# decastyle/discovering-path-tracer

Measured on AMD Instinct MI355X. Metric: Mrays/s at 1920x1080x8spp, box.obj BVH, higher is better.
Workload: dtype f32

## Files before the change

discovering-path-tracer_amd/csrc/kernels/render.h:

```cpp

__device__ __forceinline__ unsigned long long wave_sum(unsigned long long v) {
#pragma unroll
  for (int off = 32; off > 0; off >>= 1) v += __shfl_xor(v, off, 64);
  return v;
}

__device__ __forceinline__ void flush_traced(const RenderParams& P, const Ctr& c, int lane) {
  const unsigned long long v0 = wave_sum(c.rays), v1 = wave_sum(c.srays), v2 = wave_sum(c.nodes),
                           v3_ = wave_sum(c.leaves), v4 = wave_sum(c.prim);
  if (lane == 0) {
    atomicAdd(&P.stats[4], v0);
    atomicAdd(&P.stats[5], v1);
    atomicAdd(&P.stats[6], v2);
    atomicAdd(&P.stats[7], v3_);
    atomicAdd(&P.stats[8], v4);
  }
}

__device__ __forceinline__ void fold_constant(const RenderParams& P, float* acc, int spl, int j) {
  if (P.n_batches == 0) return;
#pragma unroll
  for (int ch = 0; ch < 4; ++ch) {
    if (ch % spl != j) continue;
    const float k = ch < 3 ? 0.0f : 1.0f;
    if (acc[ch] == k || (P.first_batch == 0 && __builtin_isfinite(acc[ch]))) {
      acc[ch] = k;
    } else {
      for (uint32_t t = 0; t < P.n_batches; ++t) {
        const uint32_t batch = P.first_batch + t;
        acc[ch] = (acc[ch] * (float)batch + k) / (float)(batch + 1u);
      }
    }
  }
}

__device__ __forceinline__ void store_lane(float4* px, const float* acc, int spl, int j) {
  float* a = (float*)px;
#pragma unroll
  for (int ch = 0; ch < 4; ++ch)
    if (ch % spl == j) a[ch] = acc[ch];
}

__device__ __forceinline__ void emit_lane(const RenderParams& P, bool active, size_t pix, int q, const float* acc,
                                          int spl, int j) {
  if (P.pack_out)
    store_lane(P.pack_out + (size_t)blockIdx.x * (size_t)(256 / spl) + (size_t)q, acc, spl, j);
  else if (active)
    store_lane(P.accum + pix, acc, spl, j);
}

__device__ __forceinline__ bool pixel_tight(const RenderParams& P, float ndcX0, float ndcY0) {
  if (P.n_cull_tight < 0) return true;
  bool tight = false;
#pragma unroll
  for (int r = 0; r < kMaxCullRects; ++r)
    tight = tight || (r < P.n_cull_tight && ndcX0 >= P.cull_tight[r][0] && ndcX0 <= P.cull_tight[r][1] &&
                      ndcY0 >= P.cull_tight[r][2] && ndcY0 <= P.cull_tight[r][3]);
  return tight;
}

#ifndef PT_PIX_PER_FILL
#define PT_PIX_PER_FILL 8
#endif
constexpr int kPixPerFill = PT_PIX_PER_FILL;
__device__ __forceinline__ int item_shift(int spl) { return 8 - __builtin_ctz((unsigned)spl); }
__device__ __forceinline__ void fill_culled(const RenderParams& P, const int2* __restrict__ org, int n, int block) {
  const int lg = item_shift(P.spl);
  const long long total = (long long)n << lg;
  for (int k = 0; k < kPixPerFill; ++k) {
    const long long g = ((long long)block * kPixPerFill + k) * 256 + threadIdx.x;
    if (g >= total) return;
    const int2 o = org[g >> lg];
    const int q = (int)g & ((1 << lg) - 1);
    const int px = o.x + (q & 15);
    const int py = o.y + (q >> 4);
    if (px >= P.width || py >= P.height) continue;
    float4* dst = P.accum + (size_t)py * (size_t)P.width + (size_t)px;
    float acc[4] = {0.0f, 0.0f, 0.0f, 0.0f};
    if (!(P.fresh && P.first_batch == 0)) {
      const float4 a = *dst;
      acc[0] = a.x; acc[1] = a.y; acc[2] = a.z; acc[3] = a.w;
    }
    fold_constant(P, acc, 1, 0);
    *dst = make_float4(acc[0], acc[1], acc[2], acc[3]);
  }
}

__device__ __forceinline__ bool tile_pixel(const RenderParams& P, int tile, int part, int q, size_t* pix) {
  const int spl = P.spl;
  int bx, by;
  tile_block(tile, P.blocks_x, &bx, &by);
  const int px = bx * 16 + q % 16;
  const int py = by * 16 + part * (16 / spl) + q / 16;
  *pix = (size_t)py * (size_t)P.width + (size_t)px;
  return px < P.width && py < P.height;
}

__device__ __forceinline__ void unpack_pixel(const RenderParams& P, float4* __restrict__ frame,
                                             const float4* __restrict__ src, size_t slot_f4,
                                             const int* __restrict__ table, long long g) {
  const int lg = item_shift(P.spl);
  const int4 e = ((const int4*)table)[g >> lg];
  const int q = (int)g & ((1 << lg) - 1);
  const int px = e.y + (q & 15), py = e.z + (q >> 4);
  if (px >= P.width || py >= P.height) return;
  frame[(size_t)py * (size_t)P.width + (size_t)px] =
      e.w >= 0 ? src[(size_t)e.x * slot_f4 + ((size_t)e.w << lg) + q] : make_float4(0.0f, 0.0f, 0.0f, 1.0f);
}

__device__ __forceinline__ void unpack_block(const RenderParams& P, int block) {
  const long long total = (long long)P.n_unpack * (256 / P.spl);
  for (int k = 0; k < kPixPerFill; ++k) {
    const long long g = ((long long)block * kPixPerFill + k) * 256 + threadIdx.x;
    if (g >= total) return;
    unpack_pixel(P, P.unpack_frame, P.unpack_src, (size_t)P.unpack_slot_f4, P.unpack_table, g);
  }
}

__device__ __forceinline__ float fold_one(float a, float c, uint32_t batch) {
  const float fb = (float)batch, fb1 = (float)(batch + 1u);
  if (a == 1.0f && c == 1.0f && batch < (1u << 24)) return 1.0f;
  const float x = a * fb + c;
  if (((batch + 1u) & batch) == 0u && batch + 1u != 0u) return x * (1.0f / fb1);
  return x / fb1;
}

#ifdef PT_WG_TRACE
constexpr int kWgTraceCap = 1 << 16;
__device__ unsigned long long g_wg_trace[kWgTraceCap][4];
#endif

template <bool STATS, bool LDS, bool CNT = false, int SWEEP = 0, bool MOMENTS = false, bool EXIT = false>
#ifndef PT_RENDER_MIN_BLOCKS
#define PT_RENDER_MIN_BLOCKS 5
#endif
__global__ __launch_bounds__(256, SWEEP || (LDS && !STATS) ? 6 : PT_RENDER_MIN_BLOCKS) void render_kernel(RenderParams P) {
  const int tid = (int)threadIdx.x;
  if ((P.items || P.pack_out) && (int)blockIdx.x >= P.n_items) {
    if (P.pack_out)
      unpack_block(P, (int)blockIdx.x - P.n_items);
    else
      fill_culled(P, P.culled_org, P.n_culled_items, (int)blockIdx.x - P.n_items);
    return;
  }
  const unsigned long long cost_t0 = P.cost_out ? wall_clock64() : 0ull;
  int gx0, gy0;
  bool tile_ok = true;
  int spl = P.spl;
  if (P.items_org) {
    const int2 o = P.items_org[blockIdx.x];
    gx0 = o.x & ((1 << kMixShift) - 1);
    gy0 = o.y;
    if (P.mix) spl = 1 << (o.x >> kMixShift);
  } else {
    const int item = (int)blockIdx.x;
    const int tile = rank_tile(P, item / spl);
    int bx, by;
    tile_block(tile, P.blocks_x, &bx, &by);
    gx0 = bx * 16;
    gy0 = by * 16 + (item % spl) * (16 / spl);
    tile_ok = tile < P.blocks_total;
  }
#ifdef PT_WG_TRACE
  const unsigned long long wg_t0 = wall_clock64();
#endif
  const int wave = tid >> 6, lane = tid & 63;
  static_assert(!SWEEP || (LDS && !STATS && !CNT), "the sweep walk is the plain LDS kernel's");
  constexpr int kQueue = SWEEP ? 0 : kCand;
  static_assert(!MOMENTS || (!STATS && !CNT), "moments: the plain kernels only");
  constexpr int kHand = MOMENTS ? 5 : 4;
  static_assert(kPark >= kHand, "the hand-off shares the parked state's area");
  __shared__ int cand_buf[4][kQueue + kPark][64];
  int* cand = &cand_buf[wave][0][lane];
  float* colw = (float*)&cand_buf[wave][kQueue][0];
  const int q = wave * (64 / spl) + lane / spl;
  const int j = lane % spl;
  const int px = gx0 + q % 16;
  const int py = gy0 + q / 16;
  const bool active = tile_ok && px < P.width && py < P.height;
  Ctr c = {0u, 0u, 0u, 0u, 0u};
  const int W = P.width, H = P.height;
  const float ndcX0 = (2.0f * (float)px / (float)W) - 1.0f;
  const float ndcY0 = (2.0f * (float)py / (float)H) - 1.0f;
  bool live = true;
  bool wg_live = true;
  if (P.n_cull >= 0) {
    const float wx0 = (2.0f * (float)gx0 / (float)W) - 1.0f, wx1 = (2.0f * (float)(gx0 + 15) / (float)W) - 1.0f;
    const float wy0 = (2.0f * (float)gy0 / (float)H) - 1.0f;
    const float wy1 = (2.0f * (float)(gy0 + 16 / spl - 1) / (float)H) - 1.0f;
    live = false;
    wg_live = false;
#pragma unroll
    for (int r = 0; r < kMaxCullRects; ++r) {
      live = live || (r < P.n_cull && ndcX0 >= P.cull[r][0] && ndcX0 <= P.cull[r][1] && ndcY0 >= P.cull[r][2] &&
                      ndcY0 <= P.cull[r][3]);
      wg_live = wg_live || (r < P.n_cull && wx1 >= P.cull[r][0] && wx0 <= P.cull[r][1] && wy1 >= P.cull[r][2] &&
                            wy0 <= P.cull[r][3]);
    }
  }
  const bool tight = STATS || pixel_tight(P, ndcX0, ndcY0);
  const size_t pix = (size_t)py * (size_t)W + (size_t)px;
  uint32_t nsamp = 0;
  if (active && (uint32_t)j < P.n_batches)
    nsamp = (P.n_batches - (uint32_t)j + (uint32_t)spl - 1) / (uint32_t)spl;
  float acc[4] = {0.0f, 0.0f, 0.0f, 0.0f};
  if (active && !(P.fresh && P.first_batch == 0)) {
    const float* a = (const float*)&P.accum[pix];
#pragma unroll
    for (int ch = 0; ch < 4; ++ch)
      if (ch % spl == j) acc[ch] = a[ch];
  }
  if (!live && active) fold_constant(P, acc, spl, j);
  float mom1 = 0.0f, mom2 = 0.0f;
  if constexpr (MOMENTS) {
    if (active && live && j == 0 && P.first_batch != 0) {
      const float2 m = P.moments[pix];
      mom1 = m.x;
      mom2 = m.y;
    }
  }
  if (!wg_live) {
    emit_lane(P, active, pix, q, acc, spl, j);
    return;
  }
  if (SWEEP) {
    extern __shared__ float4 lds_scene[];
    const SweepTable tb = {P.sweep, P.sweep_boxes, P.sweep_leaves};
    const int* slot = sweep_slots(tb);
    const int nt = 3 * P.sweep_leaves;
    for (int i = tid; i < nt; i += 256) lds_scene[i] = P.tris[3 * slot[i / 3] + i % 3];
    __syncthreads();
    P.tris = lds_scene;
    P.hit_tris = P.tris;
  } else if (LDS) {
    extern __shared__ float4 lds_scene[];
    const int nn = 2 * P.n_nodes, nt = 3 * P.n_tris;
    for (int i = tid; i < nn; i += 256) lds_scene[i] = P.nodes[i];
    for (int i = tid; i < nt; i += 256) lds_scene[nn + i] = P.tris[i];
    __syncthreads();
    P.nodes = lds_scene;
    P.tris = lds_scene + nn;
    P.hit_tris = P.tris;
  }
  {
    const v3 cpos = mk(P.cam_pos[0], P.cam_pos[1], P.cam_pos[2]);
    const v3 cdir = mk(P.cam_dir[0], P.cam_dir[1], P.cam_dir[2]);
    const float aspect = (float)W / (float)H;
    const v3 right = mk(P.cam_right[0], P.cam_right[1], P.cam_right[2]);
    const v3 up = mk(P.cam_upv[0], P.cam_upv[1], P.cam_upv[2]);
    const float tanFov = P.tan_fov;
    for (uint32_t base = 0; base < P.n_batches; base += (uint32_t)spl) {
     const uint32_t s = base + (uint32_t)j;
     float4 col4 = make_float4(0.0f, 0.0f, 0.0f, 1.0f);
     if (active && live && s < P.n_batches) {
      const uint32_t batch = (P.first_batch + P.seed_base) + s;
      const uint32_t seed = (batch * (uint32_t)H + (uint32_t)py) * (uint32_t)W + (uint32_t)px;
      uint32_t rng = seed;
      const float u1a = fmax_(1e-38f, rng_next(&rng));
      const float u2a = rng_next(&rng);
      const float u1j = fmax_(1e-38f, rng_next(&rng));
      const float u2j = rng_next(&rng);
      if (tight || u1a < P.cull_u0 || u1j < P.cull_u0) {
      float r = sqrt_(-2.0f * log_(u1a));
      float th = (2.0f * 0x1.921fb6p+1f) * u2a;
      float sn, cs;
      sincos_(th, &sn, &cs);
      const float ax = (r * cs) * 0.02f;
      const float ay = (r * sn) * 0.02f;
      const v3 origin = add(add(cpos, muls(right, ax)), muls(up, ay));
      r = sqrt_(-2.0f * log_(u1j));
      th = (2.0f * 0x1.921fb6p+1f) * u2j;
      sincos_(th, &sn, &cs);
      const float jx = r * cs, jy = r * sn;
      const float ndcX = ndcX0 + (jx * 0.5f) / (float)W;
      const float ndcY = ndcY0 + (jy * 0.5f) / (float)H;
      const v3 bdir = normalize(sub(add(cdir, muls(neg(right), (ndcX * tanFov) * aspect)), muls(up, ndcY * tanFov)));
      const v3 focal = add(cpos, muls(bdir, 3.0f));
      const v3 dir = normalize(sub(focal, origin));
      v3 col;
      if (CNT) c.prim++;
      if (STATS || LDS)
        col = path_trace<STATS, !LDS, CNT, SWEEP>(P, origin, dir, seed, c, cand);
      else
        col = path_trace_fused<CNT, EXIT>(P, origin, dir, seed, cand, c);
      col4 = make_float4(col.x, col.y, col.z, 1.0f);
      }
     }
     if (spl == 1) {
      if (active && live) {
        const uint32_t batch = P.first_batch + base;
        acc[0] = fold_one(acc[0], col4.x, batch);
        acc[1] = fold_one(acc[1], col4.y, batch);
        acc[2] = fold_one(acc[2], col4.z, batch);
        acc[3] = fold_one(acc[3], col4.w, batch);
        if constexpr (MOMENTS) {
          const float L = ptdn::lum(col4.x, col4.y, col4.z);
          mom1 = fold_one(mom1, L, batch);
          mom2 = fold_one(mom2, L * L, batch);
        }
      }
      continue;
     }
     colw[lane] = col4.x;
     colw[64 + lane] = col4.y;
     colw[128 + lane] = col4.z;
     colw[192 + lane] = col4.w;
     if constexpr (MOMENTS) colw[256 + lane] = ptdn::lum(col4.x, col4.y, col4.z);
     __builtin_amdgcn_fence(__ATOMIC_RELEASE, "wavefront");
     __builtin_amdgcn_wave_barrier();
     __builtin_amdgcn_fence(__ATOMIC_ACQUIRE, "wavefront");
     if (active && live) {
      const uint32_t m = min((uint32_t)spl, P.n_batches - base);
      const int first_lane = lane - j;
      for (uint32_t t = 0; t < m; ++t) {
        const uint32_t batch = P.first_batch + base + t;
        const float* cc = colw + first_lane + (int)t;
#pragma unroll
        for (int ch = 0; ch < 4; ++ch)
          if (ch % spl == j) acc[ch] = fold_one(acc[ch], cc[ch * 64], batch);
        if constexpr (MOMENTS) {
          if (j == 0) {
            const float L = cc[256];
            mom1 = fold_one(mom1, L, batch);
            mom2 = fold_one(mom2, L * L, batch);
          }
        }
      }
     }
     __builtin_amdgcn_fence(__ATOMIC_RELEASE, "wavefront");
     __builtin_amdgcn_wave_barrier();
     __builtin_amdgcn_fence(__ATOMIC_ACQUIRE, "wavefront");
    }
  }
  emit_lane(P, active, pix, q, acc, spl, j);
  if constexpr (MOMENTS) {
    if (active && live && j == 0) P.moments[pix] = make_float2(mom1, mom2);
  }
  if (!STATS && P.cost_out && lane == 0) {
    const int part_row = (gy0 + wave * (64 / spl) / 16) >> 2;
    const unsigned long long dt = wall_clock64() - cost_t0;
    atomicAdd(&P.cost_out[part_row * P.blocks_x + (gx0 >> 4)], (unsigned)(dt < 0xffffffull ? dt : 0xffffffull));
  }
#ifdef PT_WG_TRACE
  if (!STATS && !CNT) {
    __syncthreads();
    if (tid == 0 && blockIdx.x < (unsigned)kWgTraceCap) {
      const unsigned hw = __builtin_amdgcn_s_getreg((31 << 11) | 4);
      const unsigned xcc = __builtin_amdgcn_s_getreg((31 << 11) | 20);
      g_wg_trace[blockIdx.x][0] = wg_t0;
      g_wg_trace[blockIdx.x][1] = wall_clock64();
      g_wg_trace[blockIdx.x][2] = (unsigned long long)hw << 32 | (unsigned long long)((xcc & 0xff) | (spl << 8));
      g_wg_trace[blockIdx.x][3] = (unsigned long long)(unsigned)gx0 << 32 | (unsigned)gy0;
    }
  }
#endif
  if (STATS) {
    const unsigned long long rays = wave_sum(c.rays), nodes = wave_sum(c.nodes), leaves = wave_sum(c.leaves);
    const unsigned long long smp = wave_sum((unsigned long long)nsamp);
    if (lane == 0) {
      atomicAdd(&P.stats[0], rays);
      atomicAdd(&P.stats[1], nodes);
      atomicAdd(&P.stats[2], leaves);
      atomicAdd(&P.stats[3], smp);
    }
  }
  if (CNT) flush_traced(P, c, lane);
}
```

discovering-path-tracer_amd/csrc/kernels/wf_trace.h:

```cpp

template <bool CNT>
__global__ __launch_bounds__(256, 4) void wf_gen_kernel(RenderParams P, WfBuffers B, long long n, long long g0) {
  const long long g = g0 + (long long)blockIdx.x * 256 + threadIdx.x;
  bool need = false, gen = false;
  Trav T;
  PathSt S;
  if (g - g0 < n) {
    const long long pp = g / (long long)P.n_batches;
    CamFrame F;
    if (wf_pixel(P, pp, &F.px, &F.py)) {
      F.W = P.width;
      F.H = P.height;
      load_camera(P, &F.cpos, &F.cdir, &F.right, &F.up);
      F.ndcX0 = (2.0f * (float)F.px / (float)F.W) - 1.0f;
      F.ndcY0 = (2.0f * (float)F.py / (float)F.H) - 1.0f;
      F.aspect = (float)F.W / (float)F.H;
      F.tanFov = P.tan_fov;
      v3 col = mk(0.0f, 0.0f, 0.0f);
      S.s = (uint32_t)(g - pp * (long long)P.n_batches);
      bool reach = pixel_live(P, F.ndcX0, F.ndcY0);
      if (reach && !pixel_tight(P, F.ndcX0, F.ndcY0)) {
        const uint32_t batch = (P.first_batch + P.seed_base) + S.s;
        uint32_t rng = (batch * (uint32_t)F.H + (uint32_t)F.py) * (uint32_t)F.W + (uint32_t)F.px;
        const float u1a = fmax_(1e-38f, rng_next(&rng));
        rng_next(&rng);
        const float u1j = fmax_(1e-38f, rng_next(&rng));
        reach = u1a < P.cull_u0 || u1j < P.cull_u0;
      }
      if (reach) {
        gen = true;
        S.phase = PH_BEGIN;
        Ctr c = {0u, 0u, 0u, 0u, 0u};
        need = path_step<false>(P, F, S, T, c, &col);
      }
      if (!need) B.colors[g] = make_float4(col.x, col.y, col.z, 1.0f);
    }
  }
  __shared__ int wave_n[4], wave_base[4];
  const unsigned long long m = __ballot(need);
  const int w = (int)threadIdx.x >> 6, lane = (int)threadIdx.x & 63;
  if (lane == 0) wave_n[w] = (int)__popcll(m);
  __syncthreads();
  if (threadIdx.x == 0) {
    const int tot = wave_n[0] + wave_n[1] + wave_n[2] + wave_n[3];
    const int base = tot ? atomicAdd(&B.counters[0], tot) : 0;
    wave_base[0] = base;
    wave_base[1] = base + wave_n[0];
    wave_base[2] = base + wave_n[0] + wave_n[1];
    wave_base[3] = base + wave_n[0] + wave_n[1] + wave_n[2];
  }
  __syncthreads();
  const int slot =
      wave_base[w] + (int)__builtin_amdgcn_mbcnt_hi((uint32_t)(m >> 32), __builtin_amdgcn_mbcnt_lo((uint32_t)m, 0u));
  if (need) {
    wf_push(B, 0, slot, (int)g, T, fuse_bits(P, S, T), S.rng);
    wf_store_state(B, 0, slot, S);
  }
  if (CNT) {
    const unsigned long long mg = __ballot(gen);
    if (__lane_id() == 0 && mg) atomicAdd(&P.stats[8], (unsigned long long)__popcll(mg));
  }
}

struct WfLane {
  v3 o, d, inv;
  float4 a, b;
  int k, nc, res, shadow;
  float lim;
};

__device__ __forceinline__ void count_start(float4 r1, Ctr& c) {
  const int kind = __float_as_int(r1.w) & kRayKindMask;
  c.rays += kind == 0 ? 1u : 0u;
  c.srays += kind == 1 ? 1u : 0u;
}

__device__ __forceinline__ void wf_lane_start(const RenderParams& P, float4 r0, float4 r1, float4 root_a,
                                              float4 root_b, WfLane& L) {
  L.o = mk(r0.x, r0.y, r0.z);
  L.d = mk(r1.x, r1.y, r1.z);
  L.inv = mk(rcp_(L.d.x), rcp_(L.d.y), rcp_(L.d.z));
  const int kind = __float_as_int(r1.w);
  L.shadow = kind ? 1 : 0;
  L.lim = L.shadow ? r0.w : 1e30f;
  L.res = L.shadow ? 0 : -1;
  L.k = kind == 2 ? P.n_nodes : 0;
  L.nc = 0;
  L.a = root_a;
  L.b = root_b;
}

template <bool CNT = false>
__device__ __forceinline__ bool wf_lane_step(const RenderParams& P, WfLane& L, int* cand, Ctr& c) {
  if (L.k >= P.n_nodes) {
    if (!L.shadow)
      test_candidates(P, L.o, L.d, cand, L.nc, &L.lim, &L.res);
    else if (L.nc > 0)
      L.res = test_shadow_candidates(P, L.o, L.d, L.lim, cand, L.nc) ? 1 : L.res;
    return true;
  }
  if (CNT) c.nodes++;
  const int raw = __float_as_int(L.a.w);
  const bool h = slab(L.o, L.inv, L.a, L.b) || (raw < 0);
  const int tri = __float_as_int(L.b.w);
  const bool leaf_hit = h && tri >= 0;
  if (CNT) c.leaves += leaf_hit ? 1u : 0u;
  cand[L.nc * 64] = tri;
  L.nc += leaf_hit ? 1 : 0;
  const int next = (h && tri < 0) ? L.k + 1 : (raw & 0x7fffffff);
  L.a = P.nodes[2 * next];
// ... 101 lines not shown
```

discovering-path-tracer_amd/csrc/pt_api.cpp:

```cpp
#include <limits.h>
#include <math.h>
#include <stdio.h>
#include <stdlib.h>
#include <string.h>

#include <algorithm>
#include <string>
#include <vector>

#include "pt_context.h"
#include "pt_cull.h"
#include "pt_denoise.h"
#include "pt_isect.h"
#include "pt_math.h"
#include "pt_plan.h"
#include "scene/small_sweep.h"
#include "scene/threaded_bvh.h"
#include "scene/wide_bvh.h"

namespace {

thread_local std::string g_err;

std::vector<float4> as_float4(const std::vector<float>& f) {
// ... 477 lines not shown
    if (rg) return rg;
    PT_HIP(hipMemsetAsync(c->d_moments, 0, n * sizeof(float2), c->stream));
  }
  m->fold = true;
  m->cont = first_batch == 0 || (c->moments_valid && first_batch == c->moments_n);
  c->moments_valid = false;
  return PT_OK;
}
static void moments_close(pt_context* c, const Moments& m, uint32_t first_batch, uint32_t n_batches) {
  if (!m.fold) return;
  c->moments_valid = m.cont;
  c->moments_n = m.cont ? first_batch + n_batches : 0;
}

void frame_params(const pt_context* c, bool full_nodes, ptd::RenderParams* p) {
  p->nodes = full_nodes ? c->d_nodes_full : c->d_nodes;
  p->n_nodes = full_nodes ? c->n_nodes_full : c->n_nodes;
  p->tris = c->d_tris;
  p->hit_tris = c->d_tris;
  p->n_tris = c->n_tris;
  p->width = c->width;
  p->height = c->height;
  camera_params(c->cam, p);
  p->blocks_x = (c->width + 15) / 16;
  p->blocks_total = p->blocks_x * ((c->height + 15) / 16);
}

static int render_params(pt_context* c, const LaunchPlan& plan, uint32_t first_batch, uint32_t n_batches, bool packed,
                         ptd::RenderParams* p) {
  p->wf_grid = c->opt_wf_grid;
  p->wide_refill = plan.wide_refill;
  p->lights = c->d_lights_dev;
  p->accum = c->d_accum;
  p->stats = c->d_stats;
  p->n_lights = c->n_lights;
  p->first_batch = first_batch;
  p->n_batches = n_batches;
  p->seed_base = c->opt_seed_base + c->seed_extra;
  p->max_depth = c->params.max_depth;
  p->sss_bounces = c->params.sss_bounces;
  p->exit_skip = plan.exit_skip;
  memcpy(p->root_lo, c->root_lo, sizeof p->root_lo);
  memcpy(p->root_hi, c->root_hi, sizeof p->root_hi);
  p->nranks = c->nranks;
  p->rank = c->rank;
  const ptd::Part& hpart = part_of(c, c->rank);
  {
    const int rc = sync_parts(c);
    if (rc) return rc;
  }
  p->part_m = hpart.m;
  p->part_cnt = hpart.cnt;
  p->part_pos = c->d_parts + (size_t)c->rank * ptd::kMaxSlots;
  p->n_tiles = ptd::part_count(hpart, p->blocks_total);
  p->fresh = packed ? 1 : c->opt_fresh;
  p->spl = plan.spl;
  if (plan.sweep) {
    p->sweep = c->opt_sweep_hull ? c->d_sweep : c->d_sweep_plain;
    p->sweep_hull = plan.sweep_hull;
    p->sweep_boxes = c->sweep_boxes;
    p->sweep_leaves = c->sweep_leaves;
    if (plan.sweep_cube) {
      p->sweep_cube = 1;
      memcpy(p->cube_under, c->cube_under, sizeof p->cube_under);
      p->cube_all = c->cube_all;
    }
  }
  p->item_order = plan.item_order;
  return PT_OK;
}

static void cull_rectangles(const pt_context* c, ptd::RenderParams* p) {
  p->n_cull = -1;
  if (c->opt_cull && !c->stats_mode)
    p->n_cull = ptd::cull_rects(c->cam, c->width, c->height, c->root_lo, c->root_hi, c->lights_host.data(),
                                c->n_lights, &p->cull[0][0], ptd::kMaxCullRects);
  p->n_cull_tight = -1;
  p->cull_u0 = ptd::kCullTightU0;
  if (p->n_cull >= 0 && c->opt_cull_tight) {
    p->n_cull_tight = ptd::cull_rects(c->cam, c->width, c->height, c->root_lo, c->root_hi, c->lights_host.data(),
                                      c->n_lights, &p->cull_tight[0][0], ptd::kMaxCullRects, ptd::kCullTightR);
    if (p->n_cull_tight != p->n_cull) p->n_cull_tight = -1;
  }
}

static int cull_and_items(pt_context* c, const LaunchPlan& plan, uint32_t n_batches, ptd::RenderParams* p) {
  c->last_mix = 0;
  cull_rectangles(c, p);
  if (p->n_cull < 0) return PT_OK;
  MixPlan mix;
  const bool mixed = plan.mixed_eligible;
  if (mixed) {
    const size_t lds_b = plan.sweep ? ptd::sweep_lds_bytes(*p) : ptd::scene_lds_bytes(*p);
    if (c->render_slots < 0 || c->render_slots_lds != lds_b || c->render_slots_sweep != plan.sweep) {
      c->render_slots_sweep = plan.sweep;
      c->render_slots = ptd::render_slots(lds_b, plan.sweep);
      c->render_slots_lds = lds_b;
    }
    mix.budget = c->opt_mixed > 0 ? std::max(1ll, c->render_slots * c->opt_mixed / 100) : 0;
    if (c->opt_mixed < 0) {
      const int rm = mix_feedback(c, *p, n_batches);
      if (rm) return rm;
      if (c->cost_ready) {
        mix.cost = &c->block_cost;
        mix.gen = c->cost_gen;
      }
    }
  }
  const int rc = compact_items(c, p, mixed ? &mix : nullptr);
  if (rc) return rc;
  c->last_mix = !mixed || !c->items_mixed ? 0 : mix.cost ? 2 : 1;
  if (mixed && c->opt_mixed < 0 && c->cost_measure) {
    PT_HIP(hipMemsetAsync(c->d_cost, 0, (size_t)p->blocks_total * 4 * sizeof(unsigned), c->stream));
    p->cost_out = c->d_cost;
    c->cost_lanes = c->block_lanes;
  }
  return PT_OK;
}

struct Culled {
  bool launch = false, skipped = false;
};
static bool culled_hold(const pt_context* c) {
  return c->culled_state == 2 && c->culled_buf == c->d_accum && c->culled_key == c->items_key;
}
static Culled culled_before(pt_context* c, ptd::RenderParams* p, bool packed, uint32_t n_batches) {
  Culled cu;
  cu.launch = p->n_cull >= 0 && p->items && !packed && !c->stats_mode && n_batches > 0;
  if (cu.launch && culled_hold(c)) {
    p->n_culled_items = 0;
    cu.skipped = true;
  }
  return cu;
}
static void culled_after(pt_context* c, const Culled& cu, bool packed, bool fresh, uint32_t first_batch,
                         uint32_t n_batches) {
  if (cu.launch && !cu.skipped) {
    const bool exact = (fresh && first_batch == 0) || culled_hold(c) ||
                       (first_batch == 0 && c->culled_state == 1 && c->culled_buf == c->d_accum);
    c->culled_state = exact ? 2 : 0;
    c->culled_key = c->items_key;
    c->culled_buf = c->d_accum;
  } else if (!cu.launch && !packed && n_batches > 0) {
    c->culled_state = 0;
  }
}

static int assembly_params(pt_context* c, const Assembly& as, ptd::RenderParams* p) {
  if (!as.src) return PT_OK;
  const int rc = unpack_table(c, *p, c->key_scratch);
  if (rc) return rc;
  p->unpack_src = (const float4*)as.src;
  p->unpack_frame = (float4*)as.frame;
  p->unpack_table = c->d_unpack;
  p->n_unpack = c->n_unpack;
  p->unpack_slot_f4 = (long long)(as.slot_floats / 4);
  return PT_OK;
}

static int launch_wf(pt_context* c, const LaunchPlan& plan, uint32_t n_batches, ptd::RenderParams* p) {
  const long long tiles = p->n_tiles;
  const long long items = p->items ? p->n_items : tiles * p->spl;
  long long chunk_paths = 0;
  const int rc = wf_reserve(c, items * (256 / p->spl), n_batches, &chunk_paths);
  if (rc) return rc;
  ptd::WfBuffers b = c->wf;
  b.cap = chunk_paths;
  if (plan.wide) {
    const int rw = wide_params(c, p);
    if (rw) return rw;
    p->wide_handback = plan.wide_handback;
    p->wf_fuse = plan.wf_fuse;
// ... 42 lines not shown
  { const int rc = launch_wf(c, plan, n_batches, &p); if (rc) return rc; }
  { const int rc = mark_shared(c); if (rc) return rc; }
  { const int rc = timing_end(c, timer); if (rc) return rc; }
  culled_after(c, culled, false, true, 0, n_batches);
  c->packed_key = frame_k;
  const int rp = pt_items_pack(c, pack_out);
  if (rp) return rp;
  return mark_shared(c);
}

int render_impl(pt_context* c, uint32_t first_batch, uint32_t n_batches, float4* pack_out, const Assembly& as,
                Launched* launched) {
  { const int rc = render_ready(c); if (rc) return rc; }
  adaptive_forget(c);
  const bool packed = pack_out != nullptr;
  ptd::RenderParams p{};
  frame_params(c, c->stats_mode, &p);
  const LaunchPlan plan =
      plan_launch(*c, ptd::part_count(part_of(c, c->rank), p.blocks_total), n_batches, packed);
  if (plan.refuse_first) return fail(plan.refuse_code, plan.refuse);
  Moments moments;
  { const int rc = moments_open(c, first_batch, n_batches, packed, &moments); if (rc) return rc; }
  p.moments = moments.fold ? c->d_moments : nullptr;
  { const int rc = render_params(c, plan, first_batch, n_batches, packed, &p); if (rc) return rc; }
  PT_HIP(hipSetDevice(c->device));
  LaunchTimer timer;
  { const int rc = timing_begin(c, &timer); if (rc) return rc; }
  if (plan.refuse) return fail(plan.refuse_code, plan.refuse);
  { const int rc = cull_and_items(c, plan, n_batches, &p); if (rc) return rc; }
  c->last = p;
  const Culled culled = culled_before(c, &p, packed, n_batches);
  c->last_kernel = plan.wf ? 3 : 1;
  c->last_valid = true;
  if (packed && as.frame == (void*)c->d_accum) c->culled_state = 0;
  if (packed) {
    frame_key(c, p, &c->key_scratch);
    if (as.src && c->key_scratch != c->packed_key)
      return fail(PT_ERR_INVALID, "pt_render_packed: the frame to assemble has another item layout (size, partition, lanes, culling)");
    if (plan.wf) return render_packed_wavefront(c, plan, p, n_batches, pack_out, as);
    { const int rc = assembly_params(c, as, &p); if (rc) return rc; }
    if (!p.items) p.n_items = p.n_tiles * p.spl;
    c->packed_key = c->key_scratch;
    p.pack_out = pack_out;
  }
  const bool shared = !packed || plan.wf || c->stats_mode;
  if (shared) {
    const int ro = order_shared(c);
    if (ro) return ro;
  }
  if (moments.fold && first_batch == 0)
    PT_HIP(hipMemsetAsync(c->d_moments, 0, (size_t)c->width * c->height * sizeof(float2), c->stream));
  {
    const int rc = plan.wf ? launch_wf(c, plan, n_batches, &p) : launch_recursive(c, plan, p, launched);
    if (rc) return rc;
  }
  if (shared) {
    const int rm = mark_shared(c);
    if (rm) return rm;
  } else if (!c->in_dist) {
    const int ru = note_use(c);
    if (ru) return ru;
  }
  { const int rc = timing_end(c, timer); if (rc) return rc; }
  moments_close(c, moments, first_batch, n_batches);
  culled_after(c, culled, packed, c->opt_fresh != 0, first_batch, n_batches);
  return PT_OK;
}

int adaptive_render_params(pt_context* c, const AdaptivePlan& ap, int spl, ptd::RenderParams* p) {
  { const int rc = render_ready(c); if (rc) return rc; }
  if (c->n_lights < 1) return fail(PT_ERR_INVALID, "no lights uploaded");
  frame_params(c, false, p);
  LaunchPlan plan;
  plan.spl = spl;
  plan.lds = ap.lds;
  plan.exit_skip = ap.exit_skip;
  plan.sweep = ap.sweep != 0;
  plan.sweep_hull = ap.sweep >= 2;
  plan.sweep_cube = ap.sweep == 3;
  plan.wide_refill = ap.wide_refill;
  { const int rc = render_params(c, plan, 0, 0, false, p); if (rc) return rc; }
  p->moments = c->d_moments;
  cull_rectangles(c, p);
  return PT_OK;
}

int adaptive_launch_wavefront(pt_context* c, const AdaptivePlan& ap, uint32_t reserve_batches, ptd::RenderParams* p) {
  long long chunk_paths = 0;
  const int rc = wf_reserve(c, (long long)p->blocks_total * 256, reserve_batches, &chunk_paths);
  if (rc) return rc;
  ptd::WfBuffers b = c->wf;
  b.cap = chunk_paths;
  if (ap.wide) {
    const int rw = wide_params(c, p);
    if (rw) return rw;
    p->wide_handback = ap.wide_handback;
    p->wf_fuse = ap.wf_fuse;
    p->wf_tail = ap.wf_tail;
  }
  PT_HIP(ptd::launch_wavefront_adaptive(*p, b, ap.lds, c->d_ad_list, c->d_ad_live, c->stream));
  return PT_OK;
}

static void scene_release(pt_context* c) {
  dev_free(c->d_nodes);
  dev_free(c->d_nodes_full);
  dev_free(c->d_sweep);
  dev_free(c->d_sweep_plain);
  c->sweep_boxes = c->sweep_leaves = c->sweep_hull = 0;
  c->sweep_cube = false;
  dev_free(c->d_wide);
  dev_free(c->d_wide_q);
  dev_free(c->d_wide_leafbox);
  dev_free(c->d_wide_tris);
  dev_free(c->d_wide_rank_of);
  dev_free(c->d_tris);
  dev_free(c->d_wide_ovf);
  c->wide_ovf_lanes = 0;
  c->wide_ovf_stack = 0;
  c->n_wide = 0;
}

int pt_fail_internal(int code, const std::string& msg) {
  g_err = msg;
  return code;
}
void pt_note_accum_written(pt_context* c, bool finite) {
  if (!c) return;
  c->culled_state = finite ? 1 : 0;
  c->culled_buf = c->d_accum;
}

extern "C" {

int pt_abi_version(void) { return PT_ABI_VERSION; }
const char* pt_last_error(void) { return g_err.c_str(); }

int pt_create(int device_ordinal, pt_context** out) {
  if (!out) return fail(PT_ERR_INVALID, "out is null");
  *out = nullptr;
  int n = 0;
  PT_HIP(hipGetDeviceCount(&n));
  if (device_ordinal < 0 || device_ordinal >= n)
    return fail(PT_ERR_INVALID, "device ordinal " + std::to_string(device_ordinal) + " out of range (" +
                                    std::to_string(n) + " devices)");
  PT_HIP(hipSetDevice(device_ordinal));
  hipDeviceProp_t prop;
  PT_HIP(hipGetDeviceProperties(&prop, device_ordinal));
  if (strncmp(prop.gcnArchName, "gfx950", 6) != 0)
    return fail(PT_ERR_UNSUPPORTED, std::string("built for gfx950, device is ") + prop.gcnArchName);
  pt_context* c = new pt_context();
  c->device = device_ordinal;
  hipError_t e = hipStreamCreateWithFlags(&c->own_stream, hipStreamNonBlocking);
  if (e == hipSuccess) e = hipMalloc((void**)&c->d_stats, ptd::kStatsWords * sizeof(unsigned long long));
  if (e == hipSuccess) e = hipMemset(c->d_stats, 0, ptd::kStatsWords * sizeof(unsigned long long));
  for (int i = 0; i < pt_context::kRing && e == hipSuccess; ++i) {
    e = hipEventCreate(&c->ring[i][0]);
    if (e == hipSuccess) e = hipEventCreate(&c->ring[i][1]);
  }
  if (e == hipSuccess) e = hipEventCreateWithFlags(&c->shared_ev, hipEventDisableTiming);
  if (e != hipSuccess) {
    pt_destroy(c);
    return fail(PT_ERR_HIP, std::string("context setup: ") + hipGetErrorString(e));
  }
  c->stream = c->own_stream;
  *out = c;
  return PT_OK;
}

int pt_create_multi(const int* device_ordinals, int n, pt_context** out) {
  if (!out || !device_ordinals) return fail(PT_ERR_INVALID, "null argument");
  *out = nullptr;
  pt_group* g = nullptr;
  const int rc = ptg::make(device_ordinals, n, &g);
  if (rc) return rc;
  pt_context* c = new pt_context();
  c->device = device_ordinals[0];
  c->group = g;
  *out = c;
  return PT_OK;
}

int pt_group_info(pt_context* c, int* n_devices, int* devices, int max_devices, int* peer_stores) {
  if (!c) return fail(PT_ERR_INVALID, "null context");
  if (!c->group) {
    if (n_devices) *n_devices = 1;
    if (devices && max_devices > 0) devices[0] = c->device;
    if (peer_stores) *peer_stores = 0;
    return PT_OK;
  }
  return ptg::members(c->group, n_devices, devices, max_devices, peer_stores);
}

int pt_group_check(pt_context* c, int* state, float* ms_peer, float* ms_staged) {
  if (!c) return fail(PT_ERR_INVALID, "null context");
  if (!c->group) {
    if (state) *state = -1;
    if (ms_peer) *ms_peer = 0.0f;
    if (ms_staged) *ms_staged = 0.0f;
    return PT_OK;
  }
  return ptg::check_info(c->group, state, ms_peer, ms_staged);
}

int pt_destroy(pt_context* c) {
  if (!c) return PT_OK;
  if (c->group) {
    (void)ptg::destroy(c->group);
    delete c;
    return PT_OK;
  }
  (void)hipSetDevice(c->device);
  if (c->stream) (void)hipStreamSynchronize(c->stream);
  if (c->wf_stream2) (void)hipStreamSynchronize(c->wf_stream2);
  if (c->dist) (void)pt_dist_finalize(c);
  (void)quiesce(c);
  for (auto& u : c->uses) (void)hipEventDestroy(u.ev);
  c->uses.clear();
  scene_release(c);
  dev_free(c->d_lights);
  dev_free(c->d_lights_dev);
  if (c->own_accum) dev_free(c->d_accum);
  dev_free(c->d_stats);
  dev_free(c->d_items);
  dev_free(c->d_cost);
  if (c->h_cost) (void)hipHostFree(c->h_cost);
  if (c->cost_ev) (void)hipEventDestroy(c->cost_ev);
  dev_free(c->d_pack_items);
  dev_free(c->d_unpack);
  dev_free(c->d_unpack_live);
  dev_free(c->wf_block);
  dev_free(c->d_moments);
  post_release(c);
  adaptive_release(c);
  display_release(c);
  rays_release(c);
  for (auto& r : c->rb) {
    dev_free(r.dev);
    if (r.host) (void)hipHostFree(r.host);
    if (r.snap) (void)hipEventDestroy(r.snap);
    if (r.done) (void)hipEventDestroy(r.done);
  }
  if (c->copy_stream) (void)hipStreamDestroy(c->copy_stream);
  if (c->shared_ev) (void)hipEventDestroy(c->shared_ev);
  dev_free(c->d_parts);
  for (int i = 0; i < pt_context::kRing; ++i)
    for (int j = 0; j < 2; ++j)
      if (c->ring[i][j]) (void)hipEventDestroy(c->ring[i][j]);
  if (c->wf_stream2) (void)hipStreamDestroy(c->wf_stream2);
  if (c->wf_fork) (void)hipEventDestroy(c->wf_fork);
  if (c->wf_join) (void)hipEventDestroy(c->wf_join);
  if (c->own_stream) (void)hipStreamDestroy(c->own_stream);
  delete c;
  return PT_OK;
}

int pt_set_stream(pt_context* c, void* s) {
  if (c && c->group) return ptg::set_stream(c->group, s);
  if (!c) return fail(PT_ERR_INVALID, "null context");
  c->stream = s ? (hipStream_t)s : c->own_stream;
  return PT_OK;
}

int pt_synchronize(pt_context* c) {
  if (c && c->group) return ptg::synchronize(c->group);
  if (!c) return fail(PT_ERR_INVALID, "null context");
  PT_HIP(hipSetDevice(c->device));
  PT_HIP(hipStreamSynchronize(c->stream));
  return c->dist ? dist_synchronize(c) : PT_OK;
}

int pt_upload_scene(pt_context* c, const float* vertices, size_t n_vertex_floats, const uint32_t* indices,
                    size_t n_indices, const pt_bvh_node* nodes, size_t n_nodes, const float* uvs,
                    size_t n_uv_floats, const uint32_t* mat_indices, size_t n_mat, uint32_t flags) {
  if (c && c->group) return ptg::upload_scene(c->group, vertices, n_vertex_floats, indices, n_indices, nodes, n_nodes, uvs, n_uv_floats, mat_indices, n_mat, flags);
  if (!c) return fail(PT_ERR_INVALID, "null context");
  if (!vertices || !indices || !nodes) return fail(PT_ERR_INVALID, "null scene array");
  if (n_vertex_floats % 3 || n_indices % 3 || n_indices == 0)
    return fail(PT_ERR_SCENE, "vertex/index array sizes must be non-zero multiples of 3");
  if (n_nodes != 2 * (n_indices / 3) - 1)
    return fail(PT_ERR_SCENE, "expected 2T-1 = " + std::to_string(2 * (n_indices / 3) - 1) + " nodes, got " +
                                  std::to_string(n_nodes));
  if ((n_uv_floats && !uvs) || (n_mat && !mat_indices)) return fail(PT_ERR_INVALID, "null uv/material array");
  if (n_indices / 3 > 0x7fffffffull) return fail(PT_ERR_UNSUPPORTED, "too many triangles");
  const size_t nv = n_vertex_floats / 3;
  for (size_t i = 0; i < n_indices; ++i)
    if (indices[i] >= nv) return fail(PT_ERR_SCENE, "vertex index out of range at " + std::to_string(i));
  std::vector<float> threaded_f, collapsed_f;
  const std::string not_tree =
      pt::thread_bvh((const float*)nodes, n_nodes, (flags & PT_NODES_INT_BITS) != 0, n_indices / 3, &threaded_f);
  if (!not_tree.empty()) return fail(PT_ERR_SCENE, not_tree);
  pt::collapse_implied(threaded_f, &collapsed_f);
  std::vector<float4> threaded = as_float4(threaded_f), collapsed = as_float4(collapsed_f);
  pt::SmallSweep sweep;
  const bool has_sweep = pt::build_small_sweep(collapsed_f.data(), collapsed_f.size() / 8, &sweep) &&
                         (size_t)sweep.n_leaves == n_indices / 3;
  pt::WideBVH wide;
  const std::string wide_reason =
      pt::build_wide_bvh((const float*)nodes, n_nodes, (flags & PT_NODES_INT_BITS) != 0, vertices, n_vertex_floats,
                         indices, n_indices / 3, &wide, c->opt_wide_build);
  float lo[3] = {threaded[0].x, threaded[0].y, threaded[0].z};
  bool exit_normals = false;
  for (size_t t = 0; t < n_indices / 3 && !exit_normals; ++t) {
    const float* a = vertices + 3 * (size_t)indices[3 * t];
    const float* b = vertices + 3 * (size_t)indices[3 * t + 1];
    const float* d = vertices + 3 * (size_t)indices[3 * t + 2];
    const ptm::v3 v0 = ptm::mk(a[0], a[1], a[2]);
// ... 313 lines not shown
    r.host = nullptr;
    r.bytes = 0;
    PT_HIP(hipMalloc((void**)&r.dev, bytes));
    PT_HIP(hipHostMalloc(&r.host, bytes, hipHostMallocDefault));
    r.bytes = bytes;
  }
  if (!r.snap) PT_HIP(hipEventCreateWithFlags(&r.snap, hipEventDisableTiming));
  if (!r.done) PT_HIP(hipEventCreateWithFlags(&r.done, hipEventDisableTiming));
  {
    const int ro = order_shared(c);
    if (ro) return ro;
  }
  PT_HIP(hipMemcpyAsync(r.dev, c->d_accum, bytes, hipMemcpyDeviceToDevice, c->stream));
  {
    const int ru = note_use(c);
    if (ru) return ru;
  }
  PT_HIP(hipEventRecord(r.snap, c->stream));
  PT_HIP(hipStreamWaitEvent(c->copy_stream, r.snap, 0));
  PT_HIP(hipMemcpyAsync(r.host, r.dev, bytes, hipMemcpyDeviceToHost, c->copy_stream));
  PT_HIP(hipEventRecord(r.done, c->copy_stream));
  r.w = c->width;
  r.h = c->height;
  r.ticket = c->rb_next_ticket++;
  *ticket = r.ticket;
  return PT_OK;
}

int pt_readback_end(pt_context* c, int ticket, float* rgba, size_t n) {
  if (c && c->group) return ptg::readback_end(c->group, ticket, rgba, n);
  if (!c || !rgba) return fail(PT_ERR_INVALID, "null argument");
  for (auto& r : c->rb) {
    if (r.ticket != ticket || ticket == 0) continue;
    const size_t need = (size_t)r.w * r.h * 4;
    if (n < need) return fail(PT_ERR_INVALID, "output buffer too small: need " + std::to_string(need) + " floats");
    PT_HIP(hipSetDevice(c->device));
    PT_HIP(hipEventSynchronize(r.done));
    memcpy(rgba, r.host, need * sizeof(float));
    r.ticket = 0;
    return PT_OK;
  }
  return fail(PT_ERR_INVALID, "unknown or already collected readback ticket " + std::to_string(ticket));
}

int pt_last_kernel(pt_context* c, int* kernel) {
  if (c && c->group) return ptg::last_kernel(c->group, kernel);
  if (!c || !kernel) return fail(PT_ERR_INVALID, "null argument");
  *kernel = c->last_kernel;
  return PT_OK;
}

struct IntOption {
  int key;
  int pt_context::* field;
  int lo, hi;
  const char* message;
};
static const IntOption kIntOptions[] = {
    {PT_OPT_KERNEL, &pt_context::opt_kernel, 0, 3, "PT_OPT_KERNEL takes 0, 1 or 3"},
    {PT_OPT_WIDE, &pt_context::opt_wide, 0, 2, "PT_OPT_WIDE takes 0, 1 or 2"},
    {PT_OPT_WF_FUSE, &pt_context::opt_wf_fuse, 0, 1, "PT_OPT_WF_FUSE takes 0 or 1"},
    {PT_OPT_WF_TAIL, &pt_context::opt_wf_tail, -1, INT_MAX, "PT_OPT_WF_TAIL takes -1 (auto) or a ray count >= 0"},
    {PT_OPT_WF_REFILL, &pt_context::opt_wf_refill, 0, 64, "PT_OPT_WF_REFILL takes 0 (auto) to 64 idle lanes"},
    {PT_OPT_WF_GRID, &pt_context::opt_wf_grid, 1, 100, "PT_OPT_WF_GRID takes 1 to 100 (percent)"},
    {PT_OPT_WF_STREAMS, &pt_context::opt_wf_streams, 1, 2, "PT_OPT_WF_STREAMS takes 1 or 2"},
    {PT_OPT_WIDE_BUILD, &pt_context::opt_wide_build, 0, 1, "PT_OPT_WIDE_BUILD takes 0 or 1"},
    {PT_OPT_COUNT_TRACED, &pt_context::opt_count, 0, 1, "PT_OPT_COUNT_TRACED takes 0 or 1"},
    {PT_OPT_PRIMARY_CULL, &pt_context::opt_cull, 0, 1, "PT_OPT_PRIMARY_CULL takes 0 or 1"},
    {PT_OPT_WF_PATHS, &pt_context::opt_wf_paths, 0, INT_MAX, "PT_OPT_WF_PATHS takes 0 or a path count"},
    {PT_OPT_LAUNCH_TIMING, &pt_context::opt_timing, 0, INT_MAX,
     "PT_OPT_LAUNCH_TIMING takes 0 (off) or k >= 1 (every k-th launch)"},
    {PT_OPT_MIXED_LANES, &pt_context::opt_mixed, -1, 1000, "PT_OPT_MIXED_LANES takes -1 (auto), 0 (off) or 1-1000"},
    {PT_OPT_ITEM_ORDER, &pt_context::opt_item_order, -1, 1, "PT_OPT_ITEM_ORDER takes -1 (auto), 0 or 1"},
    {PT_OPT_FRESH_BATCH0, &pt_context::opt_fresh, 0, 1, "PT_OPT_FRESH_BATCH0 takes 0 or 1"},
    {PT_OPT_SCENE_IN_LDS, &pt_context::opt_scene_lds, 0, 2, "PT_OPT_SCENE_IN_LDS takes 0, 1 or 2"},
    {PT_OPT_DENOISE_LDS, &pt_context::opt_denoise_lds, 0, 1, "PT_OPT_DENOISE_LDS takes 0 or 1"},
    {PT_OPT_SMALL_SWEEP, &pt_context::opt_small_sweep, -1, 1, "PT_OPT_SMALL_SWEEP takes -1 (auto), 0 or 1"},
    {PT_OPT_CULL_TIGHT, &pt_context::opt_cull_tight, 0, 1, "PT_OPT_CULL_TIGHT takes 0 or 1"},
    {PT_OPT_SWEEP_HULL, &pt_context::opt_sweep_hull, 0, 1, "PT_OPT_SWEEP_HULL takes 0 or 1"},
    {PT_OPT_EXIT_SKIP, &pt_context::opt_exit_skip, 0, 1, "PT_OPT_EXIT_SKIP takes 0 or 1"},
    {PT_OPT_SWEEP_CUBE, &pt_context::opt_sweep_cube, 0, 1, "PT_OPT_SWEEP_CUBE takes 0 or 1"},
    {PT_OPT_ADAPTIVE_WF, &pt_context::opt_adaptive_wf, 0, 1, "PT_OPT_ADAPTIVE_WF takes 0 or 1"},
    {PT_OPT_RAYS_REFILL, &pt_context::opt_rays_refill, 0, 1, "PT_OPT_RAYS_REFILL takes 0 or 1"},
};

int pt_set_option(pt_context* c, int key, int value) {
  if (c && c->group && key == PT_OPT_MOMENTS && value != 0)
    return fail(PT_ERR_UNSUPPORTED, "PT_OPT_MOMENTS: not on a multi-device context (pt_create_multi)");
  if (c && c->group && key == PT_OPT_MOMENTS) return PT_OK;
  if (c && c->group) return ptg::set_option(c->group, key, value);
  if (!c) return fail(PT_ERR_INVALID, "null context");
  switch (key) {
    case PT_OPT_KERNEL:
      if (value == 2) return fail(PT_ERR_UNSUPPORTED, "PT_OPT_KERNEL 2 (lane state machine) was removed: slower on every scene");
      break;
    case PT_OPT_WIDE_NODE:
      if (value == 80) return fail(PT_ERR_UNSUPPORTED, "PT_OPT_WIDE_NODE 80 (8-wide nodes) was removed: slower on every scene");
      if (value != 64 && value != 128) return fail(PT_ERR_INVALID, "PT_OPT_WIDE_NODE takes 64 or 128");
      c->opt_wide_node = value;
      return PT_OK;
    case PT_OPT_PAIRS:
      if (value == 1) return fail(PT_ERR_UNSUPPORTED, "PT_OPT_PAIRS 1 (child-pair records) was removed: slower on every scene");
      if (value != 0) return fail(PT_ERR_INVALID, "PT_OPT_PAIRS takes 0");
      return PT_OK;
    case PT_OPT_SM_BATCH:
      return fail(PT_ERR_UNSUPPORTED, "PT_OPT_SM_BATCH: the lane state-machine kernel was removed");
    case PT_OPT_SAMPLE_LANES:
      if (value != 0 && value != 1 && value != 2 && value != 4 && value != 8)
        return fail(PT_ERR_INVALID, "PT_OPT_SAMPLE_LANES takes 0 (auto), 1, 2, 4 or 8");
      c->opt_sample_lanes = value;
      return PT_OK;
    case PT_OPT_MOMENTS:
      if (value != 0 && value != 1) return fail(PT_ERR_INVALID, "PT_OPT_MOMENTS takes 0 or 1");
      if (value != c->opt_moments) c->moments_valid = false;
      c->opt_moments = value;
      return PT_OK;
    case PT_OPT_SEED_BASE:
      if (value < 0) return fail(PT_ERR_INVALID, "PT_OPT_SEED_BASE takes 0 to 2^31-1");
      c->opt_seed_base = (uint32_t)value;
      return PT_OK;
    case PT_OPT_GROUP_EXCHANGE:
    case PT_OPT_GROUP_CHECK:
      return fail(PT_ERR_UNSUPPORTED, "option " + std::to_string(key) + ": multi-device contexts only (pt_create_multi)");
    default:
      break;
  }
  for (const IntOption& o : kIntOptions) {
    if (o.key != key) continue;
    if (value < o.lo || value > o.hi) return fail(PT_ERR_INVALID, o.message);
    c->*o.field = value;
    return PT_OK;
  }
  return fail(PT_ERR_INVALID, "unknown option " + std::to_string(key));
}

int pt_tiles_owned(pt_context* c, int* n_tiles) {
  PT_SINGLE(c, "pt_tiles_owned");
  if (!c || !n_tiles) return fail(PT_ERR_INVALID, "null argument");
  if (!c->d_accum) return fail(PT_ERR_INVALID, "no accumulation buffer");
  *n_tiles = ptd::owned_tiles(c->width, c->height, part_of(c, c->rank));
  return PT_OK;
}

int pt_tiles_pack(pt_context* c, void* dst) {
  PT_SINGLE(c, "pt_tiles_pack");
  if (!c || !dst) return fail(PT_ERR_INVALID, "null argument");
  if (!c->d_accum) return fail(PT_ERR_INVALID, "no accumulation buffer");
  PT_HIP(hipSetDevice(c->device));
  const int ro = order_shared(c);
  if (ro) return ro;
  {
    const int rc = sync_parts(c);
    if (rc) return rc;
  }
  PT_HIP(ptd::launch_tiles(true, c->d_accum, (float4*)dst, c->width, c->height, part_of(c, c->rank),
                           c->d_parts + (size_t)c->rank * ptd::kMaxSlots, c->stream));
  return mark_shared(c);
}

int pt_tiles_unpack(pt_context* c, const void* src, int src_rank, void* frame) {
  PT_SINGLE(c, "pt_tiles_unpack");
  if (!c || !src || !frame) return fail(PT_ERR_INVALID, "null argument");
  if (!c->d_accum) return fail(PT_ERR_INVALID, "no accumulation buffer (it sets the frame size)");
  if (src_rank < 0 || src_rank >= c->nranks) return fail(PT_ERR_INVALID, "src_rank out of range");
  if ((((uintptr_t)src) & 15) || (((uintptr_t)frame) & 15)) return fail(PT_ERR_INVALID, "buffers must be 16-B aligned");
  PT_HIP(hipSetDevice(c->device));
// ... 19 lines not shown
  *item_pixels = 256 / c->last.spl;
  return PT_OK;
}

int pt_items_pack(pt_context* c, void* dst) {
  PT_SINGLE(c, "pt_items_pack");
  if (!c || !dst) return fail(PT_ERR_INVALID, "null argument");
  if (!c->last_valid || !c->d_accum) return fail(PT_ERR_INVALID, "no path-recursive pt_render yet");
  PT_HIP(hipSetDevice(c->device));
  frame_key(c, c->last, &c->key_scratch);
  const std::vector<float>& key = c->key_scratch;
  if (key != c->pack_key) {
    std::vector<int> live, culled;
    item_lists(c->last, part_of(c, c->last.rank), &live, &culled);
    { const int rc_ = quiesce(c); if (rc_) return rc_; }
    const int rc = upload_ints(live, &c->d_pack_items, &c->pack_cap);
    if (rc) return rc;
    c->n_pack_items = (int)live.size();
    c->pack_key = key;
  }
  const int ro = order_shared(c);
  if (ro) return ro;
  PT_HIP(ptd::launch_items_pack(c->last, c->d_accum, (float4*)dst, c->d_pack_items, c->n_pack_items, c->stream));
  return mark_shared(c);
}

int pt_items_unpack_all(pt_context* c, const void* src, size_t slot_floats, void* frame) {
  PT_SINGLE(c, "pt_items_unpack_all");
  if (!c || !src || !frame) return fail(PT_ERR_INVALID, "null argument");
  if (!c->last_valid) return fail(PT_ERR_INVALID, "no path-recursive pt_render yet");
  if (c->last.first_batch != 0)
    return fail(PT_ERR_INVALID, "sparse exchange needs a frame rendered from batch 0 (culled pixels are rebuilt)");
  if ((((uintptr_t)src) & 15) || (((uintptr_t)frame) & 15) || (slot_floats & 3))
    return fail(PT_ERR_INVALID, "buffers must be 16-B aligned, slots whole float4s");
  PT_HIP(hipSetDevice(c->device));
  frame_key(c, c->last, &c->key_scratch);
  const int rc = unpack_table(c, c->last, c->key_scratch);
  if (rc) return rc;
  PT_HIP(ptd::launch_items_unpack(c->last, (float4*)frame, (const float4*)src, slot_floats / 4, c->d_unpack,
                                  c->n_unpack, c->stream));
  if (frame == (void*)c->d_accum) c->culled_state = 0;
  return note_use(c);
}

int pt_set_stats_mode(pt_context* c, int enabled) {
  if (c && c->group) return ptg::set_stats_mode(c->group, enabled);
  if (!c) return fail(PT_ERR_INVALID, "null context");
  c->stats_mode = enabled != 0;
  return PT_OK;
}

int pt_get_stats(pt_context* c, pt_stats* out) {
  if (c && c->group) return ptg::get_stats(c->group, out);
  if (!c || !out) return fail(PT_ERR_INVALID, "null argument");
  unsigned long long h[4];
  PT_HIP(hipSetDevice(c->device));
  PT_HIP(hipMemcpyAsync(h, c->d_stats, sizeof h, hipMemcpyDeviceToHost, c->stream));
  PT_HIP(hipStreamSynchronize(c->stream));
  out->rays = h[0];
  out->nodes = h[1];
  out->leaf_tests = h[2];
  out->samples = h[3];
  return PT_OK;
}

int pt_wide_info(pt_context* c, int info[2]) {
  if (c && c->group) return ptg::wide_info(c->group, info);
  if (!c || !info) return fail(PT_ERR_INVALID, "null argument");
  info[0] = c->n_wide;
  info[1] = c->n_wide ? c->wide_stack : 0;
  if (!c->n_wide) g_err = c->wide_reason;
  return PT_OK;
}

int pt_sweep_info(pt_context* c, int* boxes, int* leaves) {
  if (c && c->group) return ptg::sweep_info(c->group, boxes, leaves);
  if (!c || !boxes || !leaves) return fail(PT_ERR_INVALID, "null argument");
  const bool on = sweep_in_force(c);
  *boxes = on ? c->sweep_boxes : 0;
  *leaves = on ? c->sweep_leaves : 0;
  return PT_OK;
}

int pt_sweep_walk(pt_context* c, int* walk) {
  if (c && c->group) return ptg::sweep_walk(c->group, walk);
  if (!c || !walk) return fail(PT_ERR_INVALID, "null argument");
  *walk = sweep_in_force(c) ? sweep_walk_kind(*c) : 0;
  return PT_OK;
}

int pt_mixed_info(pt_context* c, int info[3]) {
  if (!c || !info) return fail(PT_ERR_INVALID, "null argument");
  info[0] = info[1] = info[2] = 0;
  if (c->group) return PT_OK;
  info[0] = c->last_mix;
  info[1] = c->last_mix ? c->n_live_items : 0;
  info[2] = c->cost_frames;
  return PT_OK;
}

int pt_get_traced(pt_context* c, pt_traced* out) {
  if (c && c->group) return ptg::get_traced(c->group, out);
  if (!c || !out) return fail(PT_ERR_INVALID, "null argument");
  unsigned long long h[ptd::kStatsWords];
  PT_HIP(hipSetDevice(c->device));
  PT_HIP(hipMemcpyAsync(h, c->d_stats, sizeof h, hipMemcpyDeviceToHost, c->stream));
  PT_HIP(hipStreamSynchronize(c->stream));
  out->closest_walks = h[4];
  out->shadow_walks = h[5];
  out->nodes = h[6];
  out->tri_tests = h[7];
  out->primaries = h[8];
  return PT_OK;
}

int pt_reset_stats(pt_context* c) {
  if (c && c->group) return ptg::reset_stats(c->group);
  if (!c) return fail(PT_ERR_INVALID, "null context");
  PT_HIP(hipSetDevice(c->device));
  PT_HIP(hipMemsetAsync(c->d_stats, 0, ptd::kStatsWords * sizeof(unsigned long long), c->stream));
  return note_use(c);
}

int pt_last_launch_ms(pt_context* c, float* ms) {
  if (c && c->group) return ptg::last_launch_ms(c->group, ms);
  if (!c || !ms) return fail(PT_ERR_INVALID, "null argument");
  if (!c->timed) return fail(PT_ERR_INVALID, "no launch recorded");
  PT_HIP(hipSetDevice(c->device));
  PT_HIP(hipEventSynchronize(c->ring[c->last_slot][1]));
  PT_HIP(hipEventElapsedTime(ms, c->ring[c->last_slot][0], c->ring[c->last_slot][1]));
  return PT_OK;
}

int pt_launch_times_ms(pt_context* c, float* out, size_t max_n, size_t* n_out) {
  if (c && c->group) return ptg::launch_times_ms(c->group, out, max_n, n_out);
  if (!c || !n_out) return fail(PT_ERR_INVALID, "null argument");
  const int have = c->ring_n < pt_context::kRing ? c->ring_n : pt_context::kRing;
  const int first = c->ring_n - have;
  size_t n = 0;
  PT_HIP(hipSetDevice(c->device));
  for (int k = first; k < c->ring_n && n < max_n; ++k) {
    const int slot = k % pt_context::kRing;
    PT_HIP(hipEventSynchronize(c->ring[slot][1]));
    if (out) PT_HIP(hipEventElapsedTime(&out[n], c->ring[slot][0], c->ring[slot][1]));
    ++n;
  }
  *n_out = n;
  return PT_OK;
}

int pt_launch_span_ms(pt_context* c, float* ms, size_t* n_out) {
  if (c && c->group) return ptg::launch_span_ms(c->group, ms, n_out);
  if (!c || !ms || !n_out) return fail(PT_ERR_INVALID, "null argument");
  if (c->ring_n == 0) return fail(PT_ERR_INVALID, "no launch recorded since pt_reset_launch_times");
  if (c->ring_n > pt_context::kRing) return fail(PT_ERR_UNSUPPORTED, "more launches than the event ring holds");
  PT_HIP(hipSetDevice(c->device));
  float span = 0.0f;
  for (int k = 0; k < c->ring_n; ++k) {
    float t = 0.0f;
    PT_HIP(hipEventSynchronize(c->ring[k][1]));
    PT_HIP(hipEventElapsedTime(&t, c->ring[0][0], c->ring[k][1]));
    span = t > span ? t : span;
  }
  *ms = span;
  *n_out = (size_t)(c->ring_launch[c->ring_n - 1] - c->ring_launch[0] + 1);
  return PT_OK;
// ... 98 lines not shown
```

discovering-path-tracer_amd/csrc/pt_context.h:

```cpp
#pragma once
#include <hip/hip_runtime.h>
#include <stddef.h>
#include <stdint.h>

#include <string>
#include <vector>

#include "../../include/pathtracer.h"
#include "pt_device.h"
#include "pt_group.h"

#pragma GCC visibility push(hidden)

inline int fail(int code, const std::string& msg) { return pt_fail_internal(code, msg); }

#define PT_HIP(call)                                                                   \
  do {                                                                                 \
    hipError_t e_ = (call);                                                            \
    if (e_ != hipSuccess) return fail(PT_ERR_HIP, std::string(#call ": ") + hipGetErrorString(e_)); \
  } while (0)

#define PT_SINGLE(c, name)                                                                              \
  do {                                                                                                  \
    if ((c) && (c)->group) return fail(PT_ERR_UNSUPPORTED, name ": not on a multi-device context (pt_create_multi)"); \
  } while (0)

template <class T>
void dev_free(T*& p) {
  if (p) (void)hipFree((void*)p);
  p = nullptr;
}

struct DistState;

struct pt_context {
  int device = 0;
  hipStream_t own_stream = nullptr;
  hipStream_t stream = nullptr;
  hipEvent_t shared_ev = nullptr;
  hipStream_t shared_stream = nullptr;
  struct Use {
    hipStream_t stream;
    hipEvent_t ev;
  };
  std::vector<Use> uses;

  float4* d_nodes = nullptr;
  int n_nodes = 0;
  float4* d_nodes_full = nullptr;
  int n_nodes_full = 0;
  float4* d_sweep = nullptr;
  float4* d_sweep_plain = nullptr;
  int sweep_boxes = 0, sweep_leaves = 0;
  int sweep_hull = 0;
  bool sweep_cube = false;
  uint32_t cube_under[6] = {0, 0, 0, 0, 0, 0};
  uint32_t cube_all = 0;
  float4* d_wide = nullptr;
  float4* d_wide_q = nullptr;
  float4* d_wide_leafbox = nullptr;
  float4* d_wide_tris = nullptr;
  int* d_wide_rank_of = nullptr;
  int2* d_wide_ovf = nullptr;
  long long wide_ovf_lanes = 0;
  int wide_ovf_stack = 0;
  int n_wide = 0, wide_stack = 0;
  std::string wide_reason = "no scene";
  float4* d_tris = nullptr;
  int n_tris = 0;
  float root_lo[3] = {0, 0, 0}, root_hi[3] = {0, 0, 0};
  bool exit_normals = false;
  bool has_scene = false;
  ptd::LightRec* d_lights = nullptr;
  ptd::LightDev* d_lights_dev = nullptr;
  int n_lights = 0;
  std::vector<pt_area_light> lights_host;
  int scene_serial = 0;
  float cam[16] = {0};
  bool has_camera = false;
  pt_params params{4, 3};
  float4* d_accum = nullptr;
  bool own_accum = false;
  int width = 0, height = 0;

  int opt_kernel = 0;
  int opt_scene_lds = 1;
  int opt_sample_lanes = 0;
  int opt_fresh = 0;
  int opt_item_order = -1;
  int opt_mixed = -1;
  int opt_cull = 1;
  int opt_cull_tight = 1;
  int opt_count = 0;
  int opt_small_sweep = -1;
  int opt_sweep_hull = 1;
  int opt_sweep_cube = 1;
  int opt_exit_skip = 1;
  int opt_wide = 1;
  int opt_wide_node = 64;
  int opt_wide_build = 1;
  int opt_wf_fuse = 1;
  int opt_wf_tail = -1;
  int opt_wf_grid = 100;
  int opt_wf_refill = 0;
  int opt_wf_paths = 0;
  int opt_wf_streams = 1;
  int opt_timing = 0;
  int opt_denoise_lds = 1;
  int opt_moments = 0;
  uint32_t opt_seed_base = 0;
  int opt_adaptive_wf = 0;
  int opt_rays_refill = 1;
  bool stats_mode = false;

  int nranks = 1, rank = 0;
  std::vector<int> slots{1};
  std::vector<ptd::Part> parts;
  bool parts_valid = false;
  bool parts_synced = false;
  int* d_parts = nullptr;
  size_t parts_cap = 0;
  std::vector<int> parts_key;
  int* d_items = nullptr;
  size_t items_cap = 0;
  int n_live_items = 0, n_culled_items = 0;
  bool items_mixed = false;
  std::vector<int> block_lanes;
  size_t culled_org_off = 0;
  size_t live_org_off = 0;
  std::vector<int> h_items;
  std::vector<float> items_key;
  std::vector<float> items_scratch;

  unsigned* d_cost = nullptr;
  unsigned* h_cost = nullptr;
  size_t cost_n = 0;
  hipEvent_t cost_ev = nullptr;
  bool cost_pending = false, cost_stale = false, cost_measure = false, cost_ready = false;
  int cost_stable = 0, cost_frames = 0, cost_gen = 0;
  std::vector<float> cost_key, cost_scratch;
  std::vector<int> cost_lanes;
  std::vector<double> block_cost;
  int last_mix = 0;
  long long render_slots = -1;
  size_t render_slots_lds = 0;
  bool render_slots_sweep = false;

  ptd::RenderParams last{};
  bool last_valid = false;
  int last_kernel = 0;
  int culled_state = 0;
  std::vector<float> culled_key;
  const void* culled_buf = nullptr;
  float2* d_moments = nullptr;
  size_t moments_cap = 0;
  bool moments_valid = false;
  uint32_t moments_n = 0;
  uint32_t seed_extra = 0;
  ptd::WfBuffers wf{};
  void* wf_block = nullptr;
  long long wf_fail = 0;
  hipStream_t wf_stream2 = nullptr;
  hipEvent_t wf_fork = nullptr, wf_join = nullptr;

  int* d_pack_items = nullptr;
  size_t pack_cap = 0;
  int n_pack_items = 0;
  std::vector<float> pack_key;
  int* d_unpack = nullptr;
  size_t unpack_cap = 0;
  int n_unpack = 0;
  int* d_unpack_live = nullptr;
  size_t unpack_live_cap = 0;
  int n_unpack_live = 0;
  std::vector<float> unpack_key;
  std::vector<float> packed_key;
  std::vector<float> key_scratch;

  float prog_cam[16] = {0};
  bool prog_has_cam = false;
  uint32_t prog_batch = 0;
  struct Readback {
    float4* dev = nullptr;
    void* host = nullptr;
    size_t bytes = 0;
    hipEvent_t snap = nullptr, done = nullptr;
    int ticket = 0;
    int w = 0, h = 0;
  } rb[2];
  hipStream_t copy_stream = nullptr;
  int rb_next_ticket = 1;
  unsigned long long* d_stats = nullptr;
  bool timed = false;
  static constexpr int kRing = 512;
  hipEvent_t ring[kRing][2] = {};
  int ring_n = 0;
  int last_slot = 0;
  long long launch_n = 0;
  long long ring_launch[kRing] = {};

  float4* d_guide = nullptr;
  size_t guide_cap = 0;
  bool guide_valid = false;
  float4* d_dn_scratch[2] = {nullptr, nullptr};
  size_t dn_scratch_cap[2] = {0, 0};
  float4* d_denoised = nullptr;
  size_t denoised_cap = 0;
  int denoised_w = 0, denoised_h = 0;
  float* d_var[2] = {nullptr, nullptr};
  size_t var_cap[2] = {0, 0};
  struct TemporalSet {
    float4* color = nullptr;
    float2* moments = nullptr;
    float* length = nullptr;
    float* variance = nullptr;
// ... 166 lines not shown
```

discovering-path-tracer_amd/csrc/pt_cull.cpp:

```cpp
#include <math.h>

#include "pt_context.h"
#include "pt_cull.h"

namespace {

struct D3 { double x, y, z; };
D3 d3(const float* f) { return {f[0], f[1], f[2]}; }
D3 dsub(D3 a, D3 b) { return {a.x - b.x, a.y - b.y, a.z - b.z}; }
D3 dadd(D3 a, D3 b) { return {a.x + b.x, a.y + b.y, a.z + b.z}; }
D3 dmul(D3 a, double s) { return {a.x * s, a.y * s, a.z * s}; }
double ddot(D3 a, D3 b) { return a.x * b.x + a.y * b.y + a.z * b.z; }
D3 dcross(D3 a, D3 b) { return {a.y * b.z - a.z * b.y, a.z * b.x - a.x * b.z, a.x * b.y - a.y * b.x}; }
double dlen(D3 a) { return sqrt(ddot(a, a)); }

}

int ptd::cull_rects(const float cam[16], int W, int H, const float* lo, const float* hi, const pt_area_light* lights,
                    int n_lights, float* rects, int max_rects, double Rg) {
  if (W <= 0 || H <= 0 || n_lights < 0 || n_lights + 1 > max_rects || !(Rg >= 0.0 && Rg <= kGaussR)) return -1;
  const D3 cpos = d3(cam), cdir = d3(cam + 4), cup = d3(cam + 8);
  const double fov = cam[12];
  const double L = dlen(cdir);
  if (!(L > 1e-6 && L < 1e6) || !(fov > 0.01 && fov < 170.0)) return -1;
  const D3 rx = dcross(cdir, dmul(cup, -1.0));
  const double rl = dlen(rx);
  if (!(rl > 1e-6 * L * dlen(cup))) return -1;
  const D3 right = dmul(rx, 1.0 / rl);
  const D3 ux = dcross(right, cdir);
  const D3 up = dmul(ux, 1.0 / dlen(ux));
  const D3 ez = dmul(cdir, 1.0 / L);
  const double T = tan(fov * 0.5 * M_PI / 180.0), A = (double)W / (double)H;
  const double jx = Rg * 0.5 / W, jy = Rg * 0.5 / H;
  const double amax = (1.0 + jx) * T * A / L, bmax = (1.0 + jy) * T / L;
  const double fz_min = 3.0 / sqrt(1.0 + amax * amax + bmax * bmax), fz_max = 3.0;
  const double rho = 0.02 * Rg * 1.001;
  int n = 0;
  auto add_object = [&](const D3* pts, int np) -> bool {
    double sx0 = INFINITY, sx1 = -INFINITY, sy0 = INFINITY, sy1 = -INFINITY, z0 = INFINITY, z1 = -INFINITY;
    for (int i = 0; i < np; ++i) {
      const D3 r = dsub(pts[i], cpos);
      const double X = ddot(r, right), Y = ddot(r, up), Z = ddot(r, ez);
      if (!(Z > 1e-4 * (1.0 + dlen(r)))) return false;
      sx0 = fmin(sx0, X / Z); sx1 = fmax(sx1, X / Z);
      sy0 = fmin(sy0, Y / Z); sy1 = fmax(sy1, Y / Z);
      z0 = fmin(z0, Z); z1 = fmax(z1, Z);
    }
    const double dd = fmax(fmax(fabs(1.0 / z0 - 1.0 / fz_min), fabs(1.0 / z0 - 1.0 / fz_max)),
                           fmax(fabs(1.0 / z1 - 1.0 / fz_min), fabs(1.0 / z1 - 1.0 / fz_max)));
    const double del = rho * dd;
    double x0 = -(sx1 + del) * L / (T * A), x1 = -(sx0 - del) * L / (T * A);
    double y0 = -(sy1 + del) * L / T, y1 = -(sy0 - del) * L / T;
    const double mx = 2.0 / W + 1e-4 * (1.0 + fabs(x0) + fabs(x1)), my = 2.0 / H + 1e-4 * (1.0 + fabs(y0) + fabs(y1));
    x0 -= jx + mx; x1 += jx + mx; y0 -= jy + my; y1 += jy + my;
    if (!(x0 == x0 && x1 == x1 && y0 == y0 && y1 == y1)) return false;
    float* o = rects + 4 * n++;
    o[0] = nextafterf((float)x0, -INFINITY); o[1] = nextafterf((float)x1, INFINITY);
    o[2] = nextafterf((float)y0, -INFINITY); o[3] = nextafterf((float)y1, INFINITY);
    return true;
  };
  {
    double m = 0.0;
    for (int k = 0; k < 3; ++k) m = fmax(m, fmax(fabs((double)lo[k]), fabs((double)hi[k])));
    m = 1e-4 * m + 1e-6;
    D3 pts[8];
    for (int i = 0; i < 8; ++i)
      pts[i] = {(i & 1 ? hi[0] + m : lo[0] - m), (i & 2 ? hi[1] + m : lo[1] - m), (i & 4 ? hi[2] + m : lo[2] - m)};
    if (!add_object(pts, 8)) return -1;
  }
  for (int l = 0; l < n_lights; ++l) {
    const pt_area_light& li = lights[l];
    const D3 nr = d3(li.normal);
    const double nl = dlen(nr);
    if (!(nl > 0.0)) return -1;
    const D3 nn = dmul(nr, 1.0 / nl);
    const D3 basis = fabs(nn.y) < 0.999 ? D3{0, 1, 0} : D3{1, 0, 0};
    const D3 lr = dmul(dcross(nn, basis), 1.0 / dlen(dcross(nn, basis)));
    const D3 lu = dcross(lr, nn);
    double h0 = fabs((double)li.size[0]) * 0.5, h1 = fabs((double)li.size[1]) * 0.5;
    const D3 pos = d3(li.position);
    const double pm = fmax(fmax(fabs(pos.x), fabs(pos.y)), fabs(pos.z));
    if (fabs(fabs(nn.y) - 0.999) < 1e-4) h0 = h1 = fmax(h0, h1) * 1.41422;
    h0 = h0 * 1.0001 + 1e-4 * pm + 1e-6;
    h1 = h1 * 1.0001 + 1e-4 * pm + 1e-6;
    if (!(h0 < 1e30 && h1 < 1e30)) return -1;
    D3 pts[8];
    for (int i = 0; i < 4; ++i) {
      const D3 c = dadd(dadd(pos, dmul(lr, i & 1 ? h0 : -h0)), dmul(lu, i & 2 ? h1 : -h1));
      const double th = 1e-4 * (pm + h0 + h1) + 1e-6;
      pts[2 * i] = dadd(c, dmul(nn, th));
      pts[2 * i + 1] = dadd(c, dmul(nn, -th));
    }
    if (!add_object(pts, 8)) return -1;
  }
  return n;
}

extern "C" {

int pt_primary_cull_rects(const float cam[16], int w, int h, const float root_min[3], const float root_max[3],
                          const pt_area_light* lights, int n_lights, float* rects, int max_rects, int* n_rects) {
  return pt_primary_cull_rects_r(cam, w, h, root_min, root_max, lights, n_lights, ptd::kGaussR, rects, max_rects, n_rects,
                                 nullptr);
}

int pt_primary_cull_rects_r(const float cam[16], int w, int h, const float root_min[3], const float root_max[3],
                            const pt_area_light* lights, int n_lights, double radius_bound, float* rects,
                            int max_rects, int* n_rects, float* u0) {
  if (!cam || !root_min || !root_max || !rects || !n_rects || (n_lights > 0 && !lights))
    return fail(PT_ERR_INVALID, "null argument");
  if (max_rects < 1) return fail(PT_ERR_INVALID, "max_rects must be >= 1");
  const double R = radius_bound < 0.0 ? ptd::kCullTightR : radius_bound;
  if (!(R <= ptd::kGaussR)) return fail(PT_ERR_INVALID, "radius bound above 13.25");
  *n_rects = ptd::cull_rects(cam, w, h, root_min, root_max, lights, n_lights, rects, max_rects, R);
  if (u0) *u0 = ptd::kCullTightU0;
  return PT_OK;
}

}
```

discovering-path-tracer_amd/csrc/pt_cull.h:

```cpp
#pragma once
#include "pt_math.h"

struct pt_area_light;

namespace ptd {

constexpr double kGaussR = 13.25;

#ifndef PT_CULL_TIGHT_R
#define PT_CULL_TIGHT_R 4.25
#define PT_CULL_TIGHT_U0 0x1.f5b12ep-14f
#endif
constexpr double kCullTightR = PT_CULL_TIGHT_R;

PT_FN float cull_radius(float u) { return ptm::sqrt_(-2.0f * ptm::log_(ptm::fmax_(1e-38f, u))); }

constexpr float kCullTightU0 = PT_CULL_TIGHT_U0;

__attribute__((visibility("hidden"))) int cull_rects(const float cam[16], int W, int H, const float* lo,
                                                     const float* hi, const pt_area_light* lights, int n_lights,
                                                     float* rects, int max_rects, double Rg = kGaussR);

}
```

discovering-path-tracer_amd/csrc/pt_device.h:

```cpp
#pragma once
#include <hip/hip_runtime.h>
#include <stdint.h>

namespace ptd {

struct LightRec {
  float position[4];
  float normal[4];
  float intensity[4];
  float size[4];
};

struct LightDev {
  float pos[3], nraw[3], inten[3], right[3], up[3], size[2], half[2];
  float finite;
};

__host__ __device__ inline void tile_block(int b, int blocks_x, int* bx, int* by) {
  *by = b / blocks_x;
  *bx = (b % blocks_x + *by % blocks_x) % blocks_x;
}
__host__ __device__ inline int block_tile(int bx, int by, int blocks_x) {
  return by * blocks_x + (bx - by % blocks_x + blocks_x) % blocks_x;
}

constexpr int kMaxSlots = 64;
struct Part {
  int m, cnt;
  int pos[kMaxSlots];
};
__host__ __device__ inline int part_tile(const Part& p, int li) { return (li / p.cnt) * p.m + p.pos[li % p.cnt]; }
__host__ __device__ inline int part_count(const Part& p, int total) {
  const int rem = total % p.m;
  int n = (total / p.m) * p.cnt;
  for (int i = 0; i < p.cnt; ++i) n += p.pos[i] < rem ? 1 : 0;
  return n;
}
__host__ __device__ inline bool part_owns(const Part& p, int b) {
  const int v = b % p.m;
  bool own = false;
  for (int i = 0; i < p.cnt; ++i) own = own || p.pos[i] == v;
  return own;
}

struct RenderParams {
  const float4* hit_tris;
  const float4* wide;
  int wide_qn;
  const float4* wide_leafbox;
  const float4* wide_tris;
  const int* wide_rank_of;
  int2* wide_ovf;
  long long wide_ovf_lanes;
  int wide_stack;
  int wide_handback;
  int wf_fuse;
  int wf_tail;
  int wf_grid;
  int wide_refill;
  const float4* nodes;
  const float4* tris;
  const float4* sweep = nullptr;
  int sweep_boxes = 0, sweep_leaves = 0;
  int sweep_hull = 0;
  const LightDev* lights;
  float4* accum;
  unsigned long long* stats;
  int n_nodes;
  int n_tris;
  int n_lights;
  int width, height;
  uint32_t first_batch, n_batches;
  int max_depth, sss_bounces;
  float cam_pos[3], cam_dir[3], cam_up[3], fov;
  float cam_right[3], cam_upv[3], tan_fov;
  int blocks_x, blocks_total;
  int nranks, rank;
  int part_m, part_cnt, n_tiles;
  const int* part_pos;
  int spl;
  int fresh;
  const int* items;
  const int2* items_org;
  int n_items;
  const int2* culled_org;
  int n_culled_items;
  int n_cull;
  float cull[8][4];
  int n_cull_tight = -1;
  float cull_tight[8][4] = {};
  float cull_u0 = 0.0f;
  float4* pack_out;
  const float4* unpack_src;
  float4* unpack_frame;
  const int* unpack_table;
  int n_unpack;
  long long unpack_slot_f4;
  int item_order;
  int mix = 0;
  unsigned* cost_out = nullptr;
  float2* moments = nullptr;
  int exit_skip = 0;
  float root_lo[3] = {}, root_hi[3] = {};
  uint32_t seed_base = 0;
  uint32_t cube_under[6] = {};
  uint32_t cube_all = 0;
  int sweep_cube = 0;
};
constexpr int kMixShift = 24;
constexpr int kMaxCullRects = 8;
constexpr int kStatsWords = 9;

hipError_t launch_setup_tris(const float* d_vertices, const uint32_t* d_indices, int n_tris, float4* d_tris,
                             hipStream_t stream);
hipError_t launch_setup_lights(const LightRec* d_in, int n, LightDev* d_out, hipStream_t stream);
int owned_tiles(int width, int height, const Part& part);
hipError_t launch_tiles(bool pack, float4* frame, float4* packed, int width, int height, const Part& part,
                        const int* d_pos,
                        hipStream_t stream);
hipError_t launch_clear(float4* accum, int width, int height, const Part& part, const int* d_pos, hipStream_t stream);
hipError_t launch_items_pack(const RenderParams& p, const float4* frame, float4* packed, const int* items, int n,
                             hipStream_t stream);
hipError_t launch_items_unpack(const RenderParams& p, float4* frame, const float4* src, size_t slot_f4,
                               const int* table, int n, hipStream_t stream);
constexpr size_t kMaxSceneLds = 48 * 1024;
inline size_t scene_lds_bytes(const RenderParams& p) {
  return ((size_t)2 * p.n_nodes + (size_t)3 * p.n_tris) * 16;
}
inline size_t sweep_lds_bytes(const RenderParams& p) { return (size_t)3 * p.sweep_leaves * 16; }
hipError_t launch_render(const RenderParams& p, bool stats, bool lds_scene, hipStream_t stream, bool cnt = false);
hipError_t launch_render_adaptive(const RenderParams& p, bool lds_scene, const int4* list, const int* n_live,
                                  hipStream_t stream);
struct WfBuffers {
  float4* state[2];
  float4* colors;
  int* ids[2];
  float4* rays[2];
  float2* hits;
  int* counters;
  long long cap;
};
constexpr int kWfStateF4 = 9;
constexpr int kRayKindMask = 3, kRayFuse = 4, kRayPrimary = 8;
constexpr int kHitFused = 0x40000000, kHitOccluded = 0x20000000, kHitRankMask = 0x1fffffff;
constexpr size_t kWfBytesPerPath = 2 * (size_t)kWfStateF4 * 16 + 16 + 2 * (4 + 32) + 8;
inline int wf_max_rays(const RenderParams& p) {
  return 1 + p.max_depth * (p.n_lights + p.sss_bounces * (1 + p.n_lights) + 1);
}
hipError_t launch_wavefront(const RenderParams& p, const WfBuffers& b, bool lds_scene, hipStream_t stream,
                            bool cnt = false, hipStream_t stream2 = nullptr, hipEvent_t ev_fork = nullptr,
                            hipEvent_t ev_join = nullptr);
hipError_t launch_wavefront_adaptive(const RenderParams& p, const WfBuffers& b, bool lds_scene, const int4* list,
                                     const int* n_live, hipStream_t stream);
hipError_t launch_guide(const RenderParams& p, float4* guide, bool lds_scene, hipStream_t stream);
constexpr int kRaysClosest = 0, kRaysAny = 1;
hipError_t launch_rays(const RenderParams& p, int kind, const void* rays, size_t n, void* out, uint32_t* counters,
                       const int* slot_of, bool lds_scene, bool refill, hipStream_t stream);
hipError_t launch_rays_slots(const int* rank_of, int n, int* slot_of, hipStream_t stream);
hipError_t launch_atrous(const float4* src, const float4* guide, float4* dst, int width, int height, int step,
                         float sc2, float sn2, float sz2, bool staged, hipStream_t stream);
hipError_t launch_moments_var(const float2* moments, float* var, int width, int height, uint32_t n_samples,
                              hipStream_t stream);
hipError_t launch_atrous_var(const float4* src, const float* vsrc, const float4* guide, float4* dst, float* vdst,
                             int width, int height, int step, float sigma_lum, float sn2, float sz2, bool staged,
                             hipStream_t stream);
hipError_t launch_reproject(const float4* color, const float2* moments, const float4* guide, const float4* hist_color,
                            const float2* hist_moments, const float* hist_length, const float4* hist_guide,
                            float4* out_color, float2* out_moments, float* out_length, float* out_variance,
                            const float cam_cur[16], const float cam_prev[16], int width, int height, uint32_t n,
                            uint32_t max_history, float alpha_min, float normal_min, float depth_rel,
                            hipStream_t stream);
long long wide_trace_lanes();
long long render_slots(size_t lds_bytes, bool sweep = false);
hipError_t launch_gather_tris(const float4* tris, const int* tri_of, int n, float4* dst, hipStream_t stream);
hipError_t launch_math(int fn, const float* x, float* y, size_t n, hipStream_t stream);
hipError_t launch_exhaustive(int fn, unsigned long long* bad, uint32_t* first_bad, hipStream_t stream);

#pragma GCC visibility push(hidden)
struct RenderVariant {
  bool stats, lds, cnt;
  int sweep;
  bool moments, exit;
};
struct WfTraceVariant {
  bool lds;
  int group;
  bool cnt;
};
struct WfWideVariant { bool qn, cnt; };
struct WfShadeVariant { bool exit; };
// ... 327 lines not shown
```

discovering-path-tracer_amd/csrc/pt_group.cpp:

```cpp
#include "pt_group.h"

#include <hip/hip_runtime.h>
#include <stdlib.h>
#include <string.h>

#include <algorithm>
#include <chrono>
#include <condition_variable>
#include <functional>
#include <mutex>
#include <thread>
#include <vector>

namespace {

#define G_HIP(call)                                                                             \
  do {                                                                                          \
    hipError_t e_ = (call);                                                                     \
    if (e_ != hipSuccess) return pt_fail_internal(PT_ERR_HIP, std::string(#call ": ") + hipGetErrorString(e_)); \
  } while (0)

#define G_RC(call)            \
  do {                        \
    const int rc_ = (call);   \
// ... 500 lines not shown
int progressive_advance(pt_group* g, uint32_t max_new, uint32_t limit, uint32_t* first, uint32_t* count) {
  if (!g->prog_has_cam) return pt_fail_internal(PT_ERR_INVALID, "no camera (pt_progressive_camera)");
  const uint32_t room = limit > g->prog_batch ? limit - g->prog_batch : 0u;
  const uint32_t k = max_new < room ? max_new : room;
  if (first) *first = g->prog_batch;
  if (count) *count = k;
  if (k == 0) return PT_OK;
  G_RC(render(g, g->prog_batch, k));
  g->prog_batch += k;
  return PT_OK;
}

int readback_begin(pt_group* g, int* ticket) { return pt_readback_begin(g->m[0], ticket); }
int readback_end(pt_group* g, int ticket, float* rgba, size_t n) { return pt_readback_end(g->m[0], ticket, rgba, n); }

int set_option(pt_group* g, int key, int value) {
  if (key == kOptGroupExchange) {
    if (value < 0 || value > 1) return pt_fail_internal(PT_ERR_INVALID, "PT_OPT_GROUP_EXCHANGE takes 0 or 1");
    if (value == g->exchange) return PT_OK;
    g->exchange = value;
    return g->frame ? setup_frame(g) : PT_OK;
  }
  if (key == kOptGroupCheck) {
    if (value < 0 || value > 3) return pt_fail_internal(PT_ERR_INVALID, "PT_OPT_GROUP_CHECK takes 0 to 3");
    g->check = value;
    if (value >= 2) {
      g->peer_ok = g->peer_map_ok;
      g->check_passed = false;
      return g->frame ? setup_frame(g) : PT_OK;
    }
    if (value == 0) g->check_pending = false;
    return PT_OK;
  }
  G_RC(each(g, [&](int r) { return pt_set_option(g->m[(size_t)r], key, value); }));
  if (key == kOptCountTraced) g->count_traced = value != 0;
  if (key == kOptLaunchTiming) g->timing = value;
  return PT_OK;
}

int last_kernel(pt_group* g, int* kernel) { return pt_last_kernel(g->m[0], kernel); }

int set_stats_mode(pt_group* g, int enabled) {
  G_RC(each(g, [&](int r) { return pt_set_stats_mode(g->m[(size_t)r], enabled); }));
  g->stats_mode = enabled != 0;
  return PT_OK;
}

int get_stats(pt_group* g, pt_stats* out) {
  if (!out) return pt_fail_internal(PT_ERR_INVALID, "null argument");
  pt_stats sum{};
  for (int r = 0; r < g->n; ++r) {
    pt_stats s{};
    G_RC(pt_get_stats(g->m[(size_t)r], &s));
    sum.rays += s.rays;
    sum.nodes += s.nodes;
    sum.leaf_tests += s.leaf_tests;
    sum.samples += s.samples;
  }
  *out = sum;
  return PT_OK;
}

int reset_stats(pt_group* g) { return each(g, [&](int r) { return pt_reset_stats(g->m[(size_t)r]); }); }

int get_traced(pt_group* g, pt_traced* out) {
  if (!out) return pt_fail_internal(PT_ERR_INVALID, "null argument");
  pt_traced sum{};
  for (int r = 0; r < g->n; ++r) {
    pt_traced t{};
    G_RC(pt_get_traced(g->m[(size_t)r], &t));
    sum.closest_walks += t.closest_walks;
    sum.shadow_walks += t.shadow_walks;
    sum.nodes += t.nodes;
    sum.tri_tests += t.tri_tests;
    sum.primaries += t.primaries;
  }
  *out = sum;
  return PT_OK;
}

int wide_info(pt_group* g, int info[2]) { return pt_wide_info(g->m[0], info); }
int sweep_info(pt_group* g, int* boxes, int* leaves) { return pt_sweep_info(g->m[0], boxes, leaves); }
int sweep_walk(pt_group* g, int* walk) { return pt_sweep_walk(g->m[0], walk); }
int last_launch_ms(pt_group* g, float* ms) { return pt_last_launch_ms(g->m[0], ms); }
int launch_times_ms(pt_group* g, float* out, size_t max_n, size_t* n_out) {
  return pt_launch_times_ms(g->m[0], out, max_n, n_out);
}
int launch_span_ms(pt_group* g, float* ms, size_t* n_out) { return pt_launch_span_ms(g->m[0], ms, n_out); }
int reset_launch_times(pt_group* g) {
  return each(g, [&](int r) { return pt_reset_launch_times(g->m[(size_t)r]); });
}

int members(pt_group* g, int* n, int* devices, int max_devices, int* peer) {
  if (n) *n = g->n;
  if (devices)
    for (int r = 0; r < g->n && r < max_devices; ++r) devices[r] = g->dev[(size_t)r];
  if (peer) *peer = g->n > 1 && !(g->exchange == 1 || !g->peer_ok) ? 1 : 0;
  return PT_OK;
}

int check_info(pt_group* g, int* state, float* ms_peer, float* ms_staged) {
  if (state) *state = g->check_pending ? -2 : g->check_state;
  if (ms_peer) *ms_peer = g->check_ms[0];
  if (ms_staged) *ms_staged = g->check_ms[1];
  return PT_OK;
}

}
```

discovering-path-tracer_amd/csrc/pt_group.h:

```cpp
#pragma once
#include <stddef.h>
#include <stdint.h>

#include <string>

#include "../../include/pathtracer.h"

struct pt_group;

int pt_fail_internal(int code, const std::string& msg);
void pt_note_accum_written(pt_context* c, bool finite);

namespace ptg {
int make(const int* ordinals, int n, pt_group** out);
int destroy(pt_group* g);
int set_stream(pt_group* g, void* s);
int synchronize(pt_group* g);
int upload_scene(pt_group* g, const float* vertices, size_t n_vertex_floats, const uint32_t* indices,
                 size_t n_indices, const pt_bvh_node* nodes, size_t n_nodes, const float* uvs, size_t n_uv_floats,
                 const uint32_t* mat_indices, size_t n_mat, uint32_t flags);
int upload_lights(pt_group* g, const pt_area_light* lights, size_t n);
int set_camera(pt_group* g, const float ubo[16]);
int set_params(pt_group* g, const pt_params* p);
int resize_and_clear(pt_group* g, int w, int h);
int bind_accum(pt_group* g, void* ptr, int w, int h);
int clear_accum(pt_group* g);
void* accum_device_ptr(pt_group* g);
int read_accum(pt_group* g, float* rgba, size_t n);
int render(pt_group* g, uint32_t first_batch, uint32_t n_batches);
int progressive_camera(pt_group* g, const float ubo[16], int* reset);
int progressive_advance(pt_group* g, uint32_t max_new, uint32_t limit, uint32_t* first, uint32_t* count);
int readback_begin(pt_group* g, int* ticket);
int readback_end(pt_group* g, int ticket, float* rgba, size_t n);
int set_option(pt_group* g, int key, int value);
int last_kernel(pt_group* g, int* kernel);
int set_stats_mode(pt_group* g, int enabled);
int get_stats(pt_group* g, pt_stats* out);
int reset_stats(pt_group* g);
int get_traced(pt_group* g, pt_traced* out);
int wide_info(pt_group* g, int info[2]);
int sweep_info(pt_group* g, int* boxes, int* leaves);
int sweep_walk(pt_group* g, int* walk);
int last_launch_ms(pt_group* g, float* ms);
int launch_times_ms(pt_group* g, float* out, size_t max_n, size_t* n_out);
int launch_span_ms(pt_group* g, float* ms, size_t* n_out);
int reset_launch_times(pt_group* g);
int members(pt_group* g, int* n, int* devices, int max_devices, int* peer);
int check_info(pt_group* g, int* state, float* ms_peer, float* ms_staged);
}
```

discovering-path-tracer_amd/ptamd.py:

```python
import ctypes
import os

import numpy as np

HERE = os.path.dirname(os.path.abspath(__file__))
LIB_PATH = os.environ.get("PTAMD_LIB") or os.path.join(HERE, "libptamd.so")

PT_OK = 0
PT_NODES_INT_BITS = 0x1
PT_OPT_SCENE_IN_LDS = 1
PT_OPT_SAMPLE_LANES = 2
PT_OPT_FRESH_BATCH0 = 3
PT_OPT_KERNEL = 4
PT_OPT_SM_BATCH = 5
PT_OPT_PRIMARY_CULL = 6
PT_OPT_WF_PATHS = 7
PT_OPT_ITEM_ORDER = 8
PT_OPT_LAUNCH_TIMING = 9
PT_OPT_COUNT_TRACED = 10
PT_OPT_PAIRS = 11
PT_OPT_WIDE = 12
PT_OPT_WF_STREAMS = 13
PT_OPT_WIDE_BUILD = 14
PT_OPT_WF_FUSE = 15
PT_OPT_WIDE_NODE = 16
PT_OPT_WF_TAIL = 17
PT_OPT_GROUP_EXCHANGE = 18
PT_OPT_GROUP_CHECK = 19
PT_OPT_WF_GRID = 20
PT_OPT_WF_REFILL = 21
PT_OPT_MIXED_LANES = 22
PT_OPT_DENOISE_LDS = 23
PT_OPT_SMALL_SWEEP = 24
PT_OPT_CULL_TIGHT = 25
PT_OPT_SWEEP_HULL = 26
PT_OPT_MOMENTS = 27
PT_OPT_EXIT_SKIP = 28
PT_OPT_SEED_BASE = 29
PT_OPT_SWEEP_CUBE = 30
PT_OPT_ADAPTIVE_WF = 31
PT_OPT_RAYS_REFILL = 32
RAYS_CLOSEST, RAYS_ANY = 0, 1
RAY_DTYPE = np.dtype([("o", "<f4", 3), ("d", "<f4", 3), ("limit", "<f4"), ("reserved", "<u4")])
HIT_DTYPE = np.dtype([("t", "<f4"), ("tri", "<i4"), ("u", "<f4"), ("v", "<f4"), ("n", "<f4", 3), ("reserved", "<u4")])
KERNEL_AUTO, KERNEL_RECURSIVE, KERNEL_WAVEFRONT = 0, 1, 3

EXPORTS = [
    "pt_abi_version", "pt_last_error", "pt_create", "pt_destroy", "pt_set_stream", "pt_synchronize",
    "pt_upload_scene", "pt_upload_lights", "pt_set_camera", "pt_set_params", "pt_resize_and_clear",
    "pt_bind_accum", "pt_clear_accum", "pt_accum_device_ptr", "pt_read_accum", "pt_dispatch", "pt_render",
    "pt_set_partition", "pt_tiles_owned", "pt_tiles_pack", "pt_tiles_unpack", "pt_set_option", "pt_last_kernel", "pt_set_stats_mode", "pt_get_stats", "pt_reset_stats", "pt_last_launch_ms",
    "pt_launch_times_ms", "pt_reset_launch_times", "pt_selftest_math", "pt_selftest_exhaustive",
    "pt_scene_load_obj", "pt_scene_parse_obj", "pt_scene_from_arrays", "pt_scene_build_bvh",
    "pt_scene_counts", "pt_scene_copy", "pt_scene_upload", "pt_scene_free", "pt_pack_light",
    "pt_default_camera", "pt_primary_cull_rects", "pt_primary_cull_rects_r", "pt_scene_save", "pt_scene_load_cache",
    "pt_progressive_camera", "pt_progressive_advance", "pt_readback_begin", "pt_readback_end", "pt_write_image",
    "pt_items_live", "pt_items_pack", "pt_items_unpack_all", "pt_render_packed", "pt_launch_span_ms",
    "pt_set_partition_slots", "pt_get_traced", "pt_wide_info", "pt_partition_items",
    "pt_dist_unique_id", "pt_dist_init", "pt_dist_run", "pt_dist_slot_floats", "pt_dist_finalize",
    "pt_dist_set_streams", "pt_dist_wait", "pt_dist_abort", "pt_create_multi", "pt_group_info",
    "pt_group_check", "pt_dist_info", "pt_mixed_info", "pt_sweep_info", "pt_sweep_walk",
    "pt_denoise_default_params", "pt_guide_ray", "pt_render_guide", "pt_guide_device_ptr", "pt_read_guide",
    "pt_denoise", "pt_read_denoised", "pt_denoise_host",
    "pt_moments_device_ptr", "pt_read_moments", "pt_denoise_var_default_params", "pt_denoise_var",
    "pt_denoise_var_host", "pt_denoise_var_plane_host",
    "pt_temporal_default_params", "pt_reproject", "pt_reproject_host", "pt_temporal_advance", "pt_temporal_reset",
    "pt_temporal_info", "pt_temporal_device_ptr", "pt_read_temporal", "pt_temporal_denoise",
    "pt_spatial_var_default_params", "pt_spatial_variance_host", "pt_spatial_variance", "pt_temporal_denoise_spatial",
    "pt_adaptive_default_params", "pt_adaptive_select_host", "pt_adaptive_select", "pt_adaptive_begin",
    "pt_adaptive_advance", "pt_adaptive_info", "pt_adaptive_read_counts", "pt_adaptive_read_live",
    "pt_adaptive_device_ptr", "pt_adaptive_denoise",
    "pt_display_default_params", "pt_display", "pt_display_device_ptr", "pt_read_display", "pt_display_exposure",
    "pt_display_reset", "pt_display_readback_begin", "pt_display_readback_end", "pt_display_host", "pt_write_png8",
    "pt_trace_rays", "pt_trace_rays_sync", "pt_trace_rays_host",
]


class PTError(RuntimeError):
    pass


class Params(ctypes.Structure):
    _fields_ = [("max_depth", ctypes.c_int), ("sss_bounces", ctypes.c_int)]


class Stats(ctypes.Structure):
    _fields_ = [("rays", ctypes.c_uint64), ("nodes", ctypes.c_uint64), ("leaf_tests", ctypes.c_uint64),
                ("samples", ctypes.c_uint64)]


class Traced(ctypes.Structure):
    _fields_ = [("closest_walks", ctypes.c_uint64), ("shadow_walks", ctypes.c_uint64), ("nodes", ctypes.c_uint64),
                ("tri_tests", ctypes.c_uint64), ("primaries", ctypes.c_uint64)]


class DenoiseParams(ctypes.Structure):
    _fields_ = [("iterations", ctypes.c_int), ("sigma_color", ctypes.c_float), ("sigma_normal", ctypes.c_float),
                ("sigma_depth", ctypes.c_float)]


class DenoiseVarParams(ctypes.Structure):
    _fields_ = [("iterations", ctypes.c_int), ("sigma_lum", ctypes.c_float), ("sigma_normal", ctypes.c_float),
                ("sigma_depth", ctypes.c_float)]


class TemporalParams(ctypes.Structure):
    _fields_ = [("max_history", ctypes.c_uint32), ("alpha_min", ctypes.c_float), ("normal_min", ctypes.c_float),
                ("depth_rel", ctypes.c_float)]


class SpatialVarParams(ctypes.Structure):
    _fields_ = [("below", ctypes.c_uint32), ("radius", ctypes.c_int), ("sigma_normal", ctypes.c_float),
                ("sigma_depth", ctypes.c_float)]


class AdaptiveParams(ctypes.Structure):
    _fields_ = [("min_batches", ctypes.c_uint32), ("max_batches", ctypes.c_uint32), ("step", ctypes.c_uint32),
                ("threshold", ctypes.c_float), ("lum_floor", ctypes.c_float)]


class DisplayParams(ctypes.Structure):
    _fields_ = [("tonemap", ctypes.c_int), ("exposure", ctypes.c_float), ("auto_exposure", ctypes.c_int),
                ("key", ctypes.c_float), ("white", ctypes.c_float), ("adapt", ctypes.c_float)]


TONEMAP_CLAMP, TONEMAP_REINHARD, TONEMAP_ACES = 0, 1, 2


class ReprojectImages(ctypes.Structure):
    _fields_ = [(k, ctypes.c_void_p) for k in (
        "color", "moments", "guide", "hist_color", "hist_moments", "hist_length", "hist_guide",
        "out_color", "out_moments", "out_length", "out_variance")]


_lib = None


def lib():
    global _lib
    if _lib is None:
        if not os.path.exists(LIB_PATH):
            raise PTError(f"{LIB_PATH} not built; run __graft_entry__.build() or make -C {HERE}")
        L = ctypes.CDLL(LIB_PATH)
        vp, sz, u32, i32 = ctypes.c_void_p, ctypes.c_size_t, ctypes.c_uint32, ctypes.c_int
        psz = ctypes.POINTER(sz)
        sig = {
            "pt_abi_version": ([], i32), "pt_last_error": ([], ctypes.c_char_p),
            "pt_create": ([i32, ctypes.POINTER(vp)], i32), "pt_destroy": ([vp], i32),
            "pt_create_multi": ([vp, i32, ctypes.POINTER(vp)], i32),
            "pt_group_info": ([vp, ctypes.POINTER(i32), vp, i32, ctypes.POINTER(i32)], i32),
            "pt_group_check": ([vp, ctypes.POINTER(i32), ctypes.POINTER(ctypes.c_float),
                                ctypes.POINTER(ctypes.c_float)], i32),
            "pt_dist_info": ([vp, ctypes.POINTER(i32), ctypes.POINTER(i32), ctypes.POINTER(i32)], i32),
            "pt_set_stream": ([vp, vp], i32), "pt_synchronize": ([vp], i32),
            "pt_upload_scene": ([vp, vp, sz, vp, sz, vp, sz, vp, sz, vp, sz, u32], i32),
            "pt_upload_lights": ([vp, vp, sz], i32), "pt_set_camera": ([vp, vp], i32),
            "pt_set_params": ([vp, ctypes.POINTER(Params)], i32),
            "pt_resize_and_clear": ([vp, i32, i32], i32), "pt_bind_accum": ([vp, vp, i32, i32], i32),
            "pt_clear_accum": ([vp], i32), "pt_accum_device_ptr": ([vp], vp),
            "pt_read_accum": ([vp, vp, sz], i32), "pt_dispatch": ([vp, u32], i32),
            "pt_render": ([vp, u32, u32], i32), "pt_set_partition": ([vp, i32, i32], i32),
            "pt_set_partition_slots": ([vp, i32, i32, vp], i32),
            "pt_set_stats_mode": ([vp, i32], i32), "pt_set_option": ([vp, i32, i32], i32), "pt_last_kernel": ([vp, ctypes.POINTER(ctypes.c_int)], i32),
            "pt_tiles_owned": ([vp, ctypes.POINTER(i32)], i32), "pt_tiles_pack": ([vp, vp], i32),
            "pt_tiles_unpack": ([vp, vp, i32, vp], i32), "pt_get_stats": ([vp, ctypes.POINTER(Stats)], i32),
            "pt_reset_stats": ([vp], i32), "pt_get_traced": ([vp, ctypes.POINTER(Traced)], i32),
            "pt_wide_info": ([vp, ctypes.POINTER(ctypes.c_int)], i32),
            "pt_mixed_info": ([vp, ctypes.POINTER(ctypes.c_int)], i32),
            "pt_sweep_info": ([vp, ctypes.POINTER(ctypes.c_int), ctypes.POINTER(ctypes.c_int)], i32),
            "pt_sweep_walk": ([vp, ctypes.POINTER(ctypes.c_int)], i32),
            "pt_partition_items": ([i32, i32, i32, i32, i32, vp, vp, i32, i32, vp, psz, vp, psz, vp], i32),
            "pt_dist_unique_id": ([vp, sz], i32), "pt_dist_init": ([vp, vp, i32, i32], i32),
            "pt_dist_run": ([vp, u32, i32, i32, vp, i32], i32), "pt_dist_slot_floats": ([vp, psz], i32),
            "pt_dist_finalize": ([vp], i32), "pt_dist_set_streams": ([vp, vp, vp, vp], i32),
            "pt_dist_wait": ([vp, i32], i32), "pt_dist_abort": ([vp], i32), "pt_last_launch_ms": ([vp, ctypes.POINTER(ctypes.c_float)], i32),
            "pt_launch_times_ms": ([vp, vp, sz, psz], i32), "pt_reset_launch_times": ([vp], i32),
            "pt_launch_span_ms": ([vp, ctypes.POINTER(ctypes.c_float), psz], i32),
            "pt_selftest_math": ([i32, i32, vp, vp, sz], i32),
            "pt_selftest_exhaustive": ([i32, i32, ctypes.POINTER(ctypes.c_ulonglong), ctypes.POINTER(u32)], i32),
            "pt_scene_load_obj": ([ctypes.c_char_p, ctypes.POINTER(vp)], i32),
            "pt_scene_parse_obj": ([ctypes.c_char_p, sz, ctypes.POINTER(vp)], i32),
            "pt_scene_from_arrays": ([vp, sz, vp, sz, ctypes.POINTER(vp)], i32),
            "pt_scene_build_bvh": ([vp, u32, i32], i32),
            "pt_scene_counts": ([vp, psz, psz, psz, psz, psz], i32),
            "pt_scene_copy": ([vp, vp, vp, vp, vp, vp], i32), "pt_scene_upload": ([vp, vp], i32),
            "pt_scene_free": ([vp], i32), "pt_pack_light": ([vp, vp, vp, vp, vp], i32),
            "pt_default_camera": ([vp], i32),
            "pt_primary_cull_rects": ([vp, i32, i32, vp, vp, vp, i32, vp, i32, ctypes.POINTER(i32)], i32),
            "pt_primary_cull_rects_r": ([vp, i32, i32, vp, vp, vp, i32, ctypes.c_double, vp, i32, ctypes.POINTER(i32),
                                         ctypes.POINTER(ctypes.c_float)], i32),
            "pt_scene_save": ([vp, ctypes.c_char_p], i32),
            "pt_progressive_camera": ([vp, vp, ctypes.POINTER(i32)], i32),
            "pt_progressive_advance": ([vp, u32, u32, ctypes.POINTER(u32), ctypes.POINTER(u32)], i32),
            "pt_readback_begin": ([vp, ctypes.POINTER(i32)], i32),
            "pt_readback_end": ([vp, i32, vp, sz], i32),
            "pt_write_image": ([ctypes.c_char_p, vp, i32, i32, i32], i32),
            "pt_items_live": ([vp, i32, ctypes.POINTER(i32), ctypes.POINTER(i32)], i32),
            "pt_items_pack": ([vp, vp], i32),
            "pt_items_unpack_all": ([vp, vp, sz, vp], i32),
            "pt_render_packed": ([vp, u32, vp, vp, sz, vp], i32),
            "pt_scene_load_cache": ([ctypes.c_char_p, ctypes.POINTER(vp)], i32),
            "pt_denoise_default_params": ([ctypes.POINTER(DenoiseParams)], i32),
            "pt_guide_ray": ([vp, i32, i32, i32, i32, vp, vp], i32),
            "pt_render_guide": ([vp], i32), "pt_guide_device_ptr": ([vp], vp),
            "pt_read_guide": ([vp, vp, sz], i32),
            "pt_denoise": ([vp, ctypes.POINTER(DenoiseParams), vp, vp], i32),
            "pt_read_denoised": ([vp, vp, sz], i32),
            "pt_denoise_host": ([vp, vp, i32, i32, ctypes.POINTER(DenoiseParams), vp], i32),
            "pt_moments_device_ptr": ([vp], vp),
            "pt_read_moments": ([vp, vp, sz, ctypes.POINTER(u32)], i32),
            "pt_denoise_var_default_params": ([ctypes.POINTER(DenoiseVarParams)], i32),
            "pt_denoise_var": ([vp, ctypes.POINTER(DenoiseVarParams), vp], i32),
            "pt_denoise_var_host": ([vp, vp, u32, vp, i32, i32, ctypes.POINTER(DenoiseVarParams), vp], i32),
            "pt_denoise_var_plane_host": ([vp, vp, vp, i32, i32, ctypes.POINTER(DenoiseVarParams), vp], i32),
            "pt_temporal_default_params": ([ctypes.POINTER(TemporalParams)], i32),
            "pt_reproject": ([vp, vp, vp, i32, i32, u32, ctypes.POINTER(ReprojectImages),
                              ctypes.POINTER(TemporalParams)], i32),
            "pt_reproject_host": ([vp, vp, i32, i32, u32, ctypes.POINTER(ReprojectImages),
                                   ctypes.POINTER(TemporalParams)], i32),
            "pt_temporal_advance": ([vp, vp, u32], i32), "pt_temporal_reset": ([vp], i32),
            "pt_temporal_info": ([vp, ctypes.POINTER(u32), ctypes.POINTER(u32)], i32),
            "pt_temporal_device_ptr": ([vp, i32], vp), "pt_read_temporal": ([vp, vp, vp, vp], i32),
            "pt_temporal_denoise": ([vp, ctypes.POINTER(DenoiseVarParams), vp], i32),
            "pt_spatial_var_default_params": ([ctypes.POINTER(SpatialVarParams)], i32),
            "pt_spatial_variance_host": ([vp, vp, vp, vp, i32, i32, ctypes.POINTER(SpatialVarParams), vp], i32),
            "pt_spatial_variance": ([vp, vp, vp, vp, vp, i32, i32, ctypes.POINTER(SpatialVarParams), vp], i32),
            "pt_temporal_denoise_spatial": ([vp, ctypes.POINTER(DenoiseVarParams), ctypes.POINTER(SpatialVarParams),
                                             vp], i32),
            "pt_adaptive_default_params": ([ctypes.POINTER(AdaptiveParams)], i32),
            "pt_adaptive_select_host": ([vp, vp, i32, i32, ctypes.POINTER(AdaptiveParams), vp, vp], i32),
            "pt_adaptive_select": ([vp, vp, vp, i32, i32, ctypes.POINTER(AdaptiveParams), vp, vp], i32),
            "pt_adaptive_begin": ([vp, ctypes.POINTER(AdaptiveParams)], i32),
            "pt_adaptive_advance": ([vp, u32], i32),
            "pt_adaptive_info": ([vp, ctypes.POINTER(u32), ctypes.POINTER(u32),
                                  ctypes.POINTER(ctypes.c_ulonglong)], i32),
            "pt_adaptive_read_counts": ([vp, vp, vp, sz], i32),
            "pt_adaptive_read_live": ([vp, vp, sz, ctypes.POINTER(u32)], i32),
            "pt_adaptive_device_ptr": ([vp, i32], vp),
            "pt_adaptive_denoise": ([vp, ctypes.POINTER(DenoiseVarParams), vp], i32),
            "pt_display_default_params": ([ctypes.POINTER(DisplayParams)], i32),
            "pt_display": ([vp, ctypes.POINTER(DisplayParams), vp, vp], i32),
            "pt_display_device_ptr": ([vp], vp), "pt_read_display": ([vp, vp, sz], i32),
            "pt_display_exposure": ([vp, ctypes.POINTER(ctypes.c_float), ctypes.POINTER(u32)], i32),
            "pt_display_reset": ([vp], i32),
            "pt_display_readback_begin": ([vp, ctypes.POINTER(DisplayParams), vp, ctypes.POINTER(i32)], i32),
            "pt_display_readback_end": ([vp, i32, vp, sz], i32),
            "pt_display_host": ([vp, i32, i32, ctypes.POINTER(DisplayParams), ctypes.POINTER(ctypes.c_float), vp], i32),
            "pt_write_png8": ([ctypes.c_char_p, vp, i32, i32], i32),
            "pt_trace_rays": ([vp, i32, vp, sz, vp], i32), "pt_trace_rays_sync": ([vp, i32, vp, sz, vp], i32),
            "pt_trace_rays_host": ([vp, sz, vp, sz, vp, sz, u32, i32, vp, sz, vp, i32], i32),
        }
        for name, (args, res) in sig.items():
            if not hasattr(L, name):
# ... 89 lines not shown


def reference_light():
    return pack_light([0, 2, 0], [0, -1, 0], [10, 10, 10], [2.5, 2.5])


def device_math(fn, x, device=0):
    x = np.ascontiguousarray(x, np.float32)
    y = np.empty_like(x)
    _check(lib().pt_selftest_math(device, fn, x.ctypes.data, y.ctypes.data, x.size), "pt_selftest_math")
    return y


def device_math_exhaustive(fn, device=0):
    bad = ctypes.c_ulonglong(0)
    first = ctypes.c_uint32(0)
    _check(lib().pt_selftest_exhaustive(device, fn, ctypes.byref(bad), ctypes.byref(first)),
           "pt_selftest_exhaustive")
    return bad.value, first.value


def partition_slot_positions(nranks, rank, slots=None):
    s = [1] * nranks if slots is None else [int(x) for x in slots]
    seq = sorted(((k + 0.5) / s[r], r) for r in range(nranks) for k in range(s[r]))
    return len(seq), [v for v, (_, r) in enumerate(seq) if r == rank]


def partition_owned(width, height, nranks, rank, slots=None):
    m, pos = partition_slot_positions(nranks, rank, slots)
    nbx = (width + 15) // 16
    ys, xs = np.mgrid[0:height, 0:width]
    by, bx = ys // 16, xs // 16
    return np.isin((by * nbx + (bx - by) % nbx) % m, pos)


def partition_items(width, height, sample_lanes, nranks, rank, slots=None, cull_rects=None, item_order=1):
    sl = None if slots is None else np.ascontiguousarray(slots, np.int32)
    if cull_rects is None:
        cr, nc = None, -1
    else:
        cr = np.ascontiguousarray(cull_rects, np.float32).reshape(-1, 4)
        nc = cr.shape[0]
    nl, nu = ctypes.c_size_t(0), ctypes.c_size_t(0)
    args = (width, height, sample_lanes, nranks, rank, None if sl is None else sl.ctypes.data,
            None if cr is None else cr.ctypes.data, nc, item_order)
    _check(lib().pt_partition_items(*args, None, ctypes.byref(nl), None, ctypes.byref(nu), None), "pt_partition_items")
    live = np.zeros(max(nl.value, 1), np.int32)
    culled = np.zeros(max(nu.value, 1), np.int32)
    per = 256 // sample_lanes
    pix = np.zeros(max((nl.value + nu.value) * per, 1), np.int32)
    _check(lib().pt_partition_items(*args, live.ctypes.data, ctypes.byref(nl), culled.ctypes.data, ctypes.byref(nu),
                                    pix.ctypes.data), "pt_partition_items")
    return live[:nl.value], culled[:nu.value], pix[:(nl.value + nu.value) * per].reshape(-1, per)


def primary_cull_rects(camera_ubo, width, height, root_min, root_max, lights16, max_rects=8):
    cam = np.ascontiguousarray(camera_ubo, np.float32).reshape(16)
    lo = np.ascontiguousarray(root_min, np.float32).reshape(3)
    hi = np.ascontiguousarray(root_max, np.float32).reshape(3)
    l = np.ascontiguousarray(lights16, np.float32).reshape(-1)
    out = np.zeros((max_rects, 4), np.float32)
    n = ctypes.c_int(0)
    _check(lib().pt_primary_cull_rects(cam.ctypes.data, width, height, lo.ctypes.data, hi.ctypes.data,
                                       l.ctypes.data if l.size else None, l.size // 16, out.ctypes.data,
                                       max_rects, ctypes.byref(n)), "pt_primary_cull_rects")
    return None if n.value < 0 else out[:n.value].copy()


def primary_cull_rects_r(camera_ubo, width, height, root_min, root_max, lights16, radius_bound=-1.0, max_rects=8):
    cam = np.ascontiguousarray(camera_ubo, np.float32).reshape(16)
    lo = np.ascontiguousarray(root_min, np.float32).reshape(3)
    hi = np.ascontiguousarray(root_max, np.float32).reshape(3)
    l = np.ascontiguousarray(lights16, np.float32).reshape(-1)
    out = np.zeros((max_rects, 4), np.float32)
    n = ctypes.c_int(0)
    u0 = ctypes.c_float(0.0)
    _check(lib().pt_primary_cull_rects_r(cam.ctypes.data, width, height, lo.ctypes.data, hi.ctypes.data,
                                         l.ctypes.data if l.size else None, l.size // 16, float(radius_bound),
                                         out.ctypes.data, max_rects, ctypes.byref(n), ctypes.byref(u0)),
           "pt_primary_cull_rects_r")
    return (None if n.value < 0 else out[:n.value].copy()), float(u0.value)


def write_image(path, rgba, width, height, fmt="png"):
    a = np.ascontiguousarray(rgba, np.float32).reshape(-1)
    if a.size != width * height * 4:
        raise PTError("rgba must hold width*height*4 floats")
    _check(lib().pt_write_image(str(path).encode(), a.ctypes.data, width, height, 1 if fmt == "png" else 0),
           "pt_write_image")


def write_png8(path, rgba8, width, height):
    a = np.ascontiguousarray(rgba8, np.uint8).reshape(-1)
    if a.size != width * height * 4:
        raise PTError("rgba8 must hold width*height*4 bytes")
    _check(lib().pt_write_png8(str(path).encode(), a.ctypes.data, width, height), "pt_write_png8")


def display_default_params():
    p = DisplayParams()
    _check(lib().pt_display_default_params(ctypes.byref(p)), "pt_display_default_params")
    return p


def _display_params(params):
    if params is None:
        return None
    if isinstance(params, DisplayParams):
        return ctypes.byref(params)
    tm, ex, au, key, white, adapt = params
    return ctypes.byref(DisplayParams(int(tm), float(ex), int(au), float(key), float(white), float(adapt)))


def display_host(rgba, width, height, params=None, auto_scale=0.0):
    a = np.ascontiguousarray(rgba, np.float32).reshape(-1)
    if a.size != width * height * 4:
        raise PTError("rgba must hold width*height*4 floats")
    out = np.empty(a.size, np.uint8)
    scale = ctypes.c_float(auto_scale)
    _check(lib().pt_display_host(a.ctypes.data, width, height, _display_params(params), ctypes.byref(scale),
                                 out.ctypes.data), "pt_display_host")
    return out.reshape(height, width, 4), scale.value


def default_camera():
    ubo = np.zeros(16, np.float32)
    _check(lib().pt_default_camera(ubo.ctypes.data), "pt_default_camera")
    return ubo


def denoise_default_params():
    p = DenoiseParams()
    _check(lib().pt_denoise_default_params(ctypes.byref(p)), "pt_denoise_default_params")
    return p


def _denoise_params(params):
    if params is None:
        return None
    if isinstance(params, DenoiseParams):
        return ctypes.byref(params)
    it, sc, sn, sz = params
    return ctypes.byref(DenoiseParams(int(it), float(sc), float(sn), float(sz)))


def guide_ray(camera_ubo, width, height, x, y):
    cam = np.ascontiguousarray(camera_ubo, np.float32).reshape(16)
    o, d = np.zeros(3, np.float32), np.zeros(3, np.float32)
    _check(lib().pt_guide_ray(cam.ctypes.data, width, height, x, y, o.ctypes.data, d.ctypes.data), "pt_guide_ray")
    return o, d


def denoise_host(rgba, guide, width, height, params=None):
    a = np.ascontiguousarray(rgba, np.float32).reshape(-1)
    g = np.ascontiguousarray(guide, np.float32).reshape(-1)
    if a.size != width * height * 4 or g.size != a.size:
        raise PTError("rgba and guide must hold width*height*4 floats")
    out = np.empty(a.size, np.float32)
    _check(lib().pt_denoise_host(a.ctypes.data, g.ctypes.data, width, height, _denoise_params(params),
                                 out.ctypes.data), "pt_denoise_host")
    return out.reshape(height, width, 4)


def denoise_var_default_params():
    p = DenoiseVarParams()
    _check(lib().pt_denoise_var_default_params(ctypes.byref(p)), "pt_denoise_var_default_params")
# ... 460 lines not shown
        return out.reshape(self.height, self.width, 4)

    def trace_rays(self, rays, kind=RAYS_CLOSEST):
        if type(rays).__module__.split(".")[0] == "torch":
            import torch
            if not rays.is_cuda or rays.dtype != torch.float32 or not rays.is_contiguous() or rays.numel() % 8:
                raise PTError("trace_rays: a contiguous float32 device tensor of n x 8 floats")
            n = rays.numel() // 8
            if kind not in (RAYS_CLOSEST, RAYS_ANY):
                raise PTError(f"kind is RAYS_CLOSEST or RAYS_ANY, not {kind!r}")
            out = (torch.empty((n, 8), dtype=torch.float32, device=rays.device) if kind == RAYS_CLOSEST
                   else torch.empty((n,), dtype=torch.int32, device=rays.device))
            _check(lib().pt_trace_rays(self._c, kind, rays.data_ptr() if n else None, n, out.data_ptr() if n else None),
                   "pt_trace_rays")
            return out
        r = _rays_in(rays)
        out = _rays_out(kind, r.shape[0])
        _check(lib().pt_trace_rays_sync(self._c, kind, _ptr(r), r.shape[0], _ptr(out)), "pt_trace_rays_sync")
        return out

    def set_stats_mode(self, on):
        _check(lib().pt_set_stats_mode(self._c, 1 if on else 0), "pt_set_stats_mode")

    def reset_stats(self):
        _check(lib().pt_reset_stats(self._c), "pt_reset_stats")

    def stats(self):
        s = Stats()
        _check(lib().pt_get_stats(self._c, ctypes.byref(s)), "pt_get_stats")
        return {"rays": s.rays, "nodes": s.nodes, "leaf_tests": s.leaf_tests, "samples": s.samples}

    @staticmethod
    def dist_unique_id():
        buf = (ctypes.c_char * 128)()
        _check(lib().pt_dist_unique_id(buf, 128), "pt_dist_unique_id")
        return bytes(buf)

    def dist_init(self, uid, nranks, rank):
        b = (ctypes.c_char * 128).from_buffer_copy(uid)
        _check(lib().pt_dist_init(self._c, b, nranks, rank), "pt_dist_init")

    def dist_info(self):
        c, n, r = ctypes.c_int(0), ctypes.c_int(0), ctypes.c_int(0)
        _check(lib().pt_dist_info(self._c, ctypes.byref(c), ctypes.byref(n), ctypes.byref(r)), "pt_dist_info")
        return c.value, n.value, r.value

    def dist_run(self, n_batches, n_frames, frames_ptr=None, n_frame_bufs=1, n_streams=2):
        _check(lib().pt_dist_run(self._c, n_batches, n_frames, n_streams, frames_ptr, n_frame_bufs), "pt_dist_run")

    def dist_set_streams(self, render0=None, render1=None, gather=None):
        _check(lib().pt_dist_set_streams(self._c, render0, render1, gather), "pt_dist_set_streams")

    def dist_slot_floats(self):
        n = ctypes.c_size_t(0)
        _check(lib().pt_dist_slot_floats(self._c, ctypes.byref(n)), "pt_dist_slot_floats")
        return n.value

    def dist_wait(self, timeout_ms):
        _check(lib().pt_dist_wait(self._c, timeout_ms), "pt_dist_wait")

    def dist_abort(self):
        _check(lib().pt_dist_abort(self._c), "pt_dist_abort")

    def dist_finalize(self):
        _check(lib().pt_dist_finalize(self._c), "pt_dist_finalize")

    def traced(self):
        t = Traced()
        _check(lib().pt_get_traced(self._c, ctypes.byref(t)), "pt_get_traced")
        return {k: int(getattr(t, k)) for k, _ in Traced._fields_}

    def wide_info(self):
        info = (ctypes.c_int * 2)()
        _check(lib().pt_wide_info(self._c, info), "pt_wide_info")
        if info[0] == 0:
            return 0, 0, lib().pt_last_error().decode()
        return info[0], info[1]

    def sweep_info(self):
        b, n = ctypes.c_int(0), ctypes.c_int(0)
        _check(lib().pt_sweep_info(self._c, ctypes.byref(b), ctypes.byref(n)), "pt_sweep_info")
        return b.value, n.value

    def sweep_walk(self):
        w = ctypes.c_int(0)
        _check(lib().pt_sweep_walk(self._c, ctypes.byref(w)), "pt_sweep_walk")
        return w.value

    def mixed_info(self):
        info = (ctypes.c_int * 3)()
        _check(lib().pt_mixed_info(self._c, info), "pt_mixed_info")
        return info[0], info[1], info[2]

    def last_launch_ms(self):
        ms = ctypes.c_float()
        _check(lib().pt_last_launch_ms(self._c, ctypes.byref(ms)), "pt_last_launch_ms")
        return ms.value

    def launch_times_ms(self):
        n = ctypes.c_size_t()
        out = np.zeros(512, np.float32)
        _check(lib().pt_launch_times_ms(self._c, out.ctypes.data, out.size, ctypes.byref(n)), "pt_launch_times_ms")
        return out[: n.value].copy()

    def launch_span_ms(self):
        ms, n = ctypes.c_float(), ctypes.c_size_t()
        _check(lib().pt_launch_span_ms(self._c, ctypes.byref(ms), ctypes.byref(n)), "pt_launch_span_ms")
        return ms.value, n.value

    def reset_launch_times(self):
        _check(lib().pt_reset_launch_times(self._c), "pt_reset_launch_times")

    def close(self):
        if self._c:
            lib().pt_destroy(self._c)
            self._c = None

    def __del__(self):
        try:
            self.close()
        except Exception:
            pass
```

include/pathtracer.h:

```cpp
#ifndef PATHTRACER_H_
#define PATHTRACER_H_

#include <stddef.h>
#include <stdint.h>

#ifdef __cplusplus
extern "C" {
#endif

#define PT_ABI_VERSION 3

enum {
  PT_OK = 0,
  PT_ERR_INVALID = -1,
  PT_ERR_HIP = -2,
  PT_ERR_SCENE = -3,
  PT_ERR_IO = -4,
  PT_ERR_UNSUPPORTED = -5
};

typedef struct pt_bvh_node {
  float min_bounds[4];
  float max_bounds[4];
} pt_bvh_node;
// ... 149 lines not shown
  float key;
  float white;
  float adapt;
} pt_display_params;
int pt_display_default_params(pt_display_params* out);
int pt_display(pt_context* ctx, const pt_display_params* params, const void* src_device, void* dst_device);
void* pt_display_device_ptr(pt_context* ctx);
int pt_read_display(pt_context* ctx, unsigned char* rgba8, size_t n_bytes);
int pt_display_exposure(pt_context* ctx, float* auto_scale, uint32_t* n_metered);
int pt_display_reset(pt_context* ctx);
int pt_display_readback_begin(pt_context* ctx, const pt_display_params* params, const void* src_device, int* ticket);
int pt_display_readback_end(pt_context* ctx, int ticket, unsigned char* rgba8, size_t n_bytes);
int pt_display_host(const float* rgba, int w, int h, const pt_display_params* params,
                    float* auto_scale_io, unsigned char* rgba8);

typedef struct pt_ray { float o[3]; float d[3]; float limit; uint32_t reserved; } pt_ray;
typedef struct pt_hit { float t; int32_t tri; float u, v; float n[3]; uint32_t reserved; } pt_hit;
#define PT_RAYS_CLOSEST 0
#define PT_RAYS_ANY 1
int pt_trace_rays(pt_context* ctx, int kind, const void* d_rays, size_t n, void* d_out);
int pt_trace_rays_sync(pt_context* ctx, int kind, const pt_ray* rays, size_t n, void* out);
int pt_trace_rays_host(const float* vertices, size_t n_vertex_floats, const uint32_t* indices, size_t n_indices,
                       const pt_bvh_node* nodes, size_t n_nodes, uint32_t flags, int kind, const pt_ray* rays,
                       size_t n, void* out, int threads);

int pt_set_partition(pt_context* ctx, int nranks, int rank);
int pt_set_partition_slots(pt_context* ctx, int nranks, int rank, const int* slots);
int pt_tiles_owned(pt_context* ctx, int* n_tiles);
int pt_tiles_pack(pt_context* ctx, void* dst_device);
int pt_tiles_unpack(pt_context* ctx, const void* src_device, int src_rank, void* frame_device);
int pt_items_live(pt_context* ctx, int rank, int* n_items, int* item_pixels);
int pt_items_pack(pt_context* ctx, void* dst_device);
int pt_items_unpack_all(pt_context* ctx, const void* src_device, size_t slot_floats, void* frame_device);
int pt_render_packed(pt_context* ctx, uint32_t n_batches, void* dst_device, const void* gathered_device,
                     size_t slot_floats, void* frame_device);
int pt_partition_items(int width, int height, int sample_lanes, int nranks, int rank, const int* slots,
                       const float* cull_rects, int n_cull, int item_order, int* live, size_t* n_live,
                       int* culled, size_t* n_culled, int* pixel_of);

#define PT_DIST_ID_BYTES 128
int pt_dist_unique_id(void* id, size_t id_bytes);
int pt_dist_init(pt_context* ctx, const void* id, int nranks, int rank);
int pt_dist_run(pt_context* ctx, uint32_t n_batches, int n_frames, int n_streams, void* frames_device,
                int n_frame_bufs);
int pt_dist_set_streams(pt_context* ctx, void* render_stream0, void* render_stream1, void* gather_stream);
int pt_dist_slot_floats(pt_context* ctx, size_t* slot_floats);
int pt_dist_wait(pt_context* ctx, int timeout_ms);
int pt_dist_abort(pt_context* ctx);
int pt_dist_info(pt_context* ctx, int* comm_ranks, int* nranks, int* rank);
int pt_dist_finalize(pt_context* ctx);

#define PT_OPT_SCENE_IN_LDS 1
#define PT_OPT_SAMPLE_LANES 2
#define PT_OPT_FRESH_BATCH0 3
#define PT_OPT_KERNEL 4
#define PT_OPT_SM_BATCH 5
#define PT_OPT_PRIMARY_CULL 6
#define PT_OPT_WF_PATHS 7
#define PT_OPT_ITEM_ORDER 8
#define PT_OPT_LAUNCH_TIMING 9
#define PT_OPT_COUNT_TRACED 10
#define PT_OPT_PAIRS 11
#define PT_OPT_WIDE 12
#define PT_OPT_WF_STREAMS 13
#define PT_OPT_WIDE_BUILD 14
#define PT_OPT_WF_FUSE 15
#define PT_OPT_WIDE_NODE 16
#define PT_OPT_WF_TAIL 17
#define PT_OPT_GROUP_EXCHANGE 18
#define PT_OPT_GROUP_CHECK 19
#define PT_OPT_WF_GRID 20
#define PT_OPT_WF_REFILL 21
#define PT_OPT_MIXED_LANES 22
#define PT_OPT_DENOISE_LDS 23
#define PT_OPT_SMALL_SWEEP 24
#define PT_OPT_SWEEP_HULL 26
#define PT_OPT_MOMENTS 27
#define PT_OPT_CULL_TIGHT 25
#define PT_OPT_EXIT_SKIP 28
#define PT_OPT_SEED_BASE 29
#define PT_OPT_SWEEP_CUBE 30
#define PT_OPT_ADAPTIVE_WF 31
#define PT_OPT_RAYS_REFILL 32
int pt_set_option(pt_context* ctx, int key, int value);
int pt_last_kernel(pt_context* ctx, int* kernel);

int pt_primary_cull_rects(const float camera_ubo[16], int width, int height, const float root_min[3],
                          const float root_max[3], const pt_area_light* lights, int n_lights, float* rects,
                          int max_rects, int* n_rects);
int pt_primary_cull_rects_r(const float camera_ubo[16], int width, int height, const float root_min[3],
                            const float root_max[3], const pt_area_light* lights, int n_lights, double radius_bound,
                            float* rects, int max_rects, int* n_rects, float* u0);

int pt_set_stats_mode(pt_context* ctx, int enabled);
int pt_get_stats(pt_context* ctx, pt_stats* out);
int pt_reset_stats(pt_context* ctx);
int pt_get_traced(pt_context* ctx, pt_traced* out);
int pt_wide_info(pt_context* ctx, int info[2]);
int pt_sweep_info(pt_context* ctx, int* boxes, int* leaves);
int pt_sweep_walk(pt_context* ctx, int* walk);
int pt_mixed_info(pt_context* ctx, int info[3]);
int pt_last_launch_ms(pt_context* ctx, float* ms);
int pt_launch_times_ms(pt_context* ctx, float* out, size_t max_n, size_t* n_out);
int pt_launch_span_ms(pt_context* ctx, float* ms, size_t* n_out);
int pt_reset_launch_times(pt_context* ctx);
int pt_selftest_math(int device_ordinal, int fn, const float* x, float* y, size_t n);
int pt_selftest_exhaustive(int device, int fn, unsigned long long* mismatches, uint32_t* first_bad);

typedef struct pt_scene pt_scene;
int pt_scene_load_obj(const char* path, pt_scene** out);
int pt_scene_parse_obj(const char* text, size_t len, pt_scene** out);
int pt_scene_from_arrays(const float* vertices, size_t n_vertex_floats,
                         const uint32_t* indices, size_t n_indices, pt_scene** out);
int pt_scene_build_bvh(pt_scene* scene, uint32_t flags, int threads);
int pt_scene_counts(const pt_scene* scene, size_t* n_vertex_floats, size_t* n_indices,
                    size_t* n_nodes, size_t* n_uv_floats, size_t* n_mat);
int pt_scene_copy(const pt_scene* scene, float* vertices, uint32_t* indices, pt_bvh_node* nodes,
                  float* uvs, uint32_t* mat_indices);
int pt_scene_upload(pt_context* ctx, const pt_scene* scene);
int pt_scene_free(pt_scene* scene);
int pt_scene_save(const pt_scene* scene, const char* path);
int pt_scene_load_cache(const char* path, pt_scene** out);
int pt_pack_light(const float position[3], const float normal[3], const float intensity[3],
                  const float size[2], pt_area_light* out);
#define PT_IMAGE_PFM 0
#define PT_IMAGE_PNG 1
int pt_write_image(const char* path, const float* rgba, int width, int height, int format);
int pt_write_png8(const char* path, const unsigned char* rgba8, int width, int height);
int pt_default_camera(float camera_ubo[16]);

#ifdef __cplusplus
}
#endif
#endif
```

Measured before the change: 266,500.

## Cull primary rays with convex-hull footprints and shade sure-light pixels directly

Replaces the rectangular tight-cull test with per-object convex footprints (a rectangle plus up to four half-planes) computed on the host from the camera, scene root box and area lights, uploaded to a small device table only when it changes. Pixels outside every footprint are known to be black, so their rays are skipped. Pixels lying in a 'sure' region that falls entirely inside a single light get that light's emitted intensity without tracing. This cuts path-tracing work for more pixels in exchange for extra per-pixel region tests and a more intricate conservative-bounds computation, which must stay exact to keep the image correct.

```diff
diff --git a/discovering-path-tracer_amd/csrc/kernels/render.h b/discovering-path-tracer_amd/csrc/kernels/render.h
--- a/discovering-path-tracer_amd/csrc/kernels/render.h
+++ b/discovering-path-tracer_amd/csrc/kernels/render.h
@@ -49,14 +49,50 @@
     store_lane(P.accum + pix, acc, spl, j);
 }
 
-__device__ __forceinline__ bool pixel_tight(const RenderParams& P, float ndcX0, float ndcY0) {
-  if (P.n_cull_tight < 0) return true;
+__device__ __forceinline__ bool region_holds(const float* __restrict__ f, float x, float y) {
+  bool in = x >= f[0] && x <= f[1] && y >= f[2] && y <= f[3];
+#pragma unroll
+  for (int k = 0; k < kFootprintPlanes; ++k) in = in && f[4 + 3 * k] * x + f[5 + 3 * k] * y <= f[6 + 3 * k];
+  return in;
+}
+
+constexpr int kSkipNever = -2, kSkipBlack = -1;
+__device__ __forceinline__ int pixel_skip(const RenderParams& P, float ndcX0, float ndcY0) {
+  if (P.n_cull_tight < 0) return kSkipNever;
+  if (P.n_foot > 0) {
+    int inside = 0, last = 0;
+    for (int r = 0; r < P.n_foot; ++r) {
+      const bool in = region_holds(P.foot + kFootprintFloats * r, ndcX0, ndcY0);
+      inside += in ? 1 : 0;
+      last = in ? r : last;
+    }
+    if (inside == 0) return kSkipBlack;
+    if (inside == 1 && last >= 1 && last <= P.n_sure &&
+        region_holds(P.foot + kFootprintFloats * (kMaxCullRects + last - 1), ndcX0, ndcY0))
+      return last - 1;
+    return kSkipNever;
+  }
   bool tight = false;
 #pragma unroll
   for (int r = 0; r < kMaxCullRects; ++r)
     tight = tight || (r < P.n_cull_tight && ndcX0 >= P.cull_tight[r][0] && ndcX0 <= P.cull_tight[r][1] &&
                       ndcY0 >= P.cull_tight[r][2] && ndcY0 <= P.cull_tight[r][3]);
-  return tight;
+  return tight ? kSkipNever : kSkipBlack;
+}
+__device__ __forceinline__ bool pixel_tight(const RenderParams& P, float ndcX0, float ndcY0) {
+  return pixel_skip(P, ndcX0, ndcY0) != kSkipBlack;
+}
+__device__ __forceinline__ int skip_again(const RenderParams& P, float ndcX0, float ndcY0) {
+  asm volatile("" : "+v"(ndcX0), "+v"(ndcY0));
+  int l = 0;
+  for (int k = 1; k < P.n_sure; ++k)
+    l = region_holds(P.foot + kFootprintFloats * (kMaxCullRects + k), ndcX0, ndcY0) ? k : l;
+  return l;
+}
+__device__ __forceinline__ float4 skip_colour(const RenderParams& P, int skip) {
+  if (skip < 0) return make_float4(0.0f, 0.0f, 0.0f, 1.0f);
+  const LightDev* L = P.lights + skip;
+  return make_float4(L->inten[0], L->inten[1], L->inten[2], 1.0f);
 }
 
 #ifndef PT_PIX_PER_FILL
@@ -198,7 +234,9 @@
                             wy0 <= P.cull[r][3]);
     }
   }
-  const bool tight = STATS || pixel_tight(P, ndcX0, ndcY0);
+  const int skip0 = STATS ? kSkipNever : pixel_skip(P, ndcX0, ndcY0);
+  const bool tight = skip0 == kSkipNever;
+  const bool sure = skip0 >= 0;
   const size_t pix = (size_t)py * (size_t)W + (size_t)px;
   uint32_t nsamp = 0;
   if (active && (uint32_t)j < P.n_batches)
@@ -284,6 +322,8 @@
       else
         col = path_trace_fused<CNT, EXIT>(P, origin, dir, seed, cand, c);
       col4 = make_float4(col.x, col.y, col.z, 1.0f);
+      } else if (sure) {
+        col4 = skip_colour(P, skip_again(P, ndcX0, ndcY0));
       }
      }
      if (spl == 1) {
diff --git a/discovering-path-tracer_amd/csrc/kernels/wf_trace.h b/discovering-path-tracer_amd/csrc/kernels/wf_trace.h
--- a/discovering-path-tracer_amd/csrc/kernels/wf_trace.h
+++ b/discovering-path-tracer_amd/csrc/kernels/wf_trace.h
@@ -19,13 +19,18 @@
       v3 col = mk(0.0f, 0.0f, 0.0f);
       S.s = (uint32_t)(g - pp * (long long)P.n_batches);
       bool reach = pixel_live(P, F.ndcX0, F.ndcY0);
-      if (reach && !pixel_tight(P, F.ndcX0, F.ndcY0)) {
+      const int skip = reach ? pixel_skip(P, F.ndcX0, F.ndcY0) : kSkipBlack;
+      if (reach && skip != kSkipNever) {
         const uint32_t batch = (P.first_batch + P.seed_base) + S.s;
         uint32_t rng = (batch * (uint32_t)F.H + (uint32_t)F.py) * (uint32_t)F.W + (uint32_t)F.px;
         const float u1a = fmax_(1e-38f, rng_next(&rng));
         rng_next(&rng);
         const float u1j = fmax_(1e-38f, rng_next(&rng));
         reach = u1a < P.cull_u0 || u1j < P.cull_u0;
+        if (!reach) {
+          const float4 c4 = skip_colour(P, skip);
+          col = mk(c4.x, c4.y, c4.z);
+        }
       }
       if (reach) {
         gen = true;
diff --git a/discovering-path-tracer_amd/csrc/pt_api.cpp b/discovering-path-tracer_amd/csrc/pt_api.cpp
--- a/discovering-path-tracer_amd/csrc/pt_api.cpp
+++ b/discovering-path-tracer_amd/csrc/pt_api.cpp
@@ -583,12 +583,54 @@
                                       c->n_lights, &p->cull_tight[0][0], ptd::kMaxCullRects, ptd::kCullTightR);
     if (p->n_cull_tight != p->n_cull) p->n_cull_tight = -1;
   }
+  p->n_foot = 0;
+  p->n_sure = 0;
+  p->foot = nullptr;
+}
+
+constexpr size_t kFootTable = 2 * (size_t)ptd::kMaxCullRects * ptd::kFootprintFloats;
+static_assert(ptd::kMaxCullObjects == ptd::kMaxCullRects, "pt_cull.h's bound is pt_device.h's");
+static int cull_footprint_table(const pt_context* c, const ptd::RenderParams& p, float* table, int* n_sure,
+                                int* sure_regions) {
+  *n_sure = *sure_regions = 0;
+  const bool counting = c->opt_count != 0 && !c->stats_mode;
+  if (p.n_cull_tight < 1 || c->opt_cull_foot == 0 || (c->opt_cull_foot < 0 && counting)) return 0;
+  const int n = ptd::cull_footprints(c->cam, c->width, c->height, c->root_lo, c->root_hi, c->lights_host.data(),
+                                     c->n_lights, table, ptd::kMaxCullRects, ptd::kCullTightR);
+  if (n != p.n_cull_tight) return 0;
+  const int ns = ptd::cull_sure(c->cam, c->width, c->height, c->root_lo, c->root_hi, c->lights_host.data(), c->n_lights,
+                                table + ptd::kMaxCullRects * ptd::kFootprintFloats, ptd::kMaxCullRects, ptd::kCullTightR);
+  if (ns > 0) {
+    *n_sure = c->n_lights;
+    *sure_regions = ns;
+  }
+  return n;
+}
+
+static int cull_footprints(pt_context* c, ptd::RenderParams* p) {
+  static_assert(sizeof(c->foot_up) == kFootTable * sizeof(float), "pt_context::foot_up");
+  float table[kFootTable] = {};
+  int n_sure = 0, regions = 0;
+  const int n = cull_footprint_table(c, *p, table, &n_sure, &regions);
+  if (n == 0) return PT_OK;
+  if (!c->d_foot || memcmp(table, c->foot_up, sizeof(table)) != 0) {
+    { const int rc_ = quiesce(c); if (rc_) return rc_; }
+    PT_HIP(hipSetDevice(c->device));
+    if (!c->d_foot) PT_HIP(hipMalloc((void**)&c->d_foot, sizeof(table)));
+    PT_HIP(hipMemcpy(c->d_foot, table, sizeof(table), hipMemcpyHostToDevice));
+    memcpy(c->foot_up, table, sizeof(table));
+  }
+  p->n_foot = n;
+  p->n_sure = n_sure;
+  p->foot = c->d_foot;
+  return PT_OK;
 }
 
 static int cull_and_items(pt_context* c, const LaunchPlan& plan, uint32_t n_batches, ptd::RenderParams* p) {
   c->last_mix = 0;
   cull_rectangles(c, p);
   if (p->n_cull < 0) return PT_OK;
+  { const int rc = cull_footprints(c, p); if (rc) return rc; }
   MixPlan mix;
   const bool mixed = plan.mixed_eligible;
   if (mixed) {
@@ -797,7 +839,7 @@
   { const int rc = render_params(c, plan, 0, 0, false, p); if (rc) return rc; }
   p->moments = c->d_moments;
   cull_rectangles(c, p);
-  return PT_OK;
+  return cull_footprints(c, p);
 }
 
 int adaptive_launch_wavefront(pt_context* c, const AdaptivePlan& ap, uint32_t reserve_batches, ptd::RenderParams* p) {
@@ -938,6 +980,7 @@
   if (c->own_accum) dev_free(c->d_accum);
   dev_free(c->d_stats);
   dev_free(c->d_items);
+  dev_free(c->d_foot);
   dev_free(c->d_cost);
   if (c->h_cost) (void)hipHostFree(c->h_cost);
   if (c->cost_ev) (void)hipEventDestroy(c->cost_ev);
@@ -1417,6 +1460,7 @@
     {PT_OPT_SWEEP_CUBE, &pt_context::opt_sweep_cube, 0, 1, "PT_OPT_SWEEP_CUBE takes 0 or 1"},
     {PT_OPT_ADAPTIVE_WF, &pt_context::opt_adaptive_wf, 0, 1, "PT_OPT_ADAPTIVE_WF takes 0 or 1"},
     {PT_OPT_RAYS_REFILL, &pt_context::opt_rays_refill, 0, 1, "PT_OPT_RAYS_REFILL takes 0 or 1"},
+    {PT_OPT_CULL_FOOTPRINT, &pt_context::opt_cull_foot, -1, 1, "PT_OPT_CULL_FOOTPRINT takes -1 (auto), 0 or 1"},
 };
 
 int pt_set_option(pt_context* c, int key, int value) {
@@ -1602,6 +1646,18 @@
   return PT_OK;
 }
 
+int pt_cull_info(pt_context* c, int info[3]) {
+  if (c && c->group) return ptg::cull_info(c->group, info);
+  if (!c || !info) return fail(PT_ERR_INVALID, "null argument");
+  ptd::RenderParams p{};
+  cull_rectangles(c, &p);
+  float table[kFootTable];
+  int n_sure = 0;
+  info[0] = p.n_cull_tight > 0 ? p.n_cull_tight : 0;
+  info[1] = cull_footprint_table(c, p, table, &n_sure, &info[2]);
+  return PT_OK;
+}
+
 int pt_sweep_walk(pt_context* c, int* walk) {
   if (c && c->group) return ptg::sweep_walk(c->group, walk);
   if (!c || !walk) return fail(PT_ERR_INVALID, "null argument");
diff --git a/discovering-path-tracer_amd/csrc/pt_context.h b/discovering-path-tracer_amd/csrc/pt_context.h
--- a/discovering-path-tracer_amd/csrc/pt_context.h
+++ b/discovering-path-tracer_amd/csrc/pt_context.h
@@ -91,6 +91,7 @@
   int opt_mixed = -1;
   int opt_cull = 1;
   int opt_cull_tight = 1;
+  int opt_cull_foot = -1;
   int opt_count = 0;
   int opt_small_sweep = -1;
   int opt_sweep_hull = 1;
@@ -131,6 +132,8 @@
   std::vector<int> h_items;
   std::vector<float> items_key;
   std::vector<float> items_scratch;
+  float* d_foot = nullptr;
+  float foot_up[2 * ptd::kMaxCullRects * 16] = {};
 
   unsigned* d_cost = nullptr;
   unsigned* h_cost = nullptr;
diff --git a/discovering-path-tracer_amd/csrc/pt_cull.cpp b/discovering-path-tracer_amd/csrc/pt_cull.cpp
--- a/discovering-path-tracer_amd/csrc/pt_cull.cpp
+++ b/discovering-path-tracer_amd/csrc/pt_cull.cpp
@@ -14,85 +14,312 @@
 D3 dcross(D3 a, D3 b) { return {a.y * b.z - a.z * b.y, a.z * b.x - a.x * b.z, a.x * b.y - a.y * b.x}; }
 double dlen(D3 a) { return sqrt(ddot(a, a)); }
 
-}
-
-int ptd::cull_rects(const float cam[16], int W, int H, const float* lo, const float* hi, const pt_area_light* lights,
-                    int n_lights, float* rects, int max_rects, double Rg) {
-  if (W <= 0 || H <= 0 || n_lights < 0 || n_lights + 1 > max_rects || !(Rg >= 0.0 && Rg <= kGaussR)) return -1;
-  const D3 cpos = d3(cam), cdir = d3(cam + 4), cup = d3(cam + 8);
+struct CullFrame {
+  D3 cpos, right, up, ez;
+  double L, T, A, jx, jy, fz_min, fz_max, rho;
+};
+
+bool cull_frame(const float cam[16], int W, int H, double Rg, CullFrame* f) {
+  if (W <= 0 || H <= 0 || !(Rg >= 0.0 && Rg <= ptd::kGaussR)) return false;
+  const D3 cdir = d3(cam + 4), cup = d3(cam + 8);
+  f->cpos = d3(cam);
   const double fov = cam[12];
   const double L = dlen(cdir);
-  if (!(L > 1e-6 && L < 1e6) || !(fov > 0.01 && fov < 170.0)) return -1;
+  if (!(L > 1e-6 && L < 1e6) || !(fov > 0.01 && fov < 170.0)) return false;
   const D3 rx = dcross(cdir, dmul(cup, -1.0));
   const double rl = dlen(rx);
-  if (!(rl > 1e-6 * L * dlen(cup))) return -1;
-  const D3 right = dmul(rx, 1.0 / rl);
-  const D3 ux = dcross(right, cdir);
-  const D3 up = dmul(ux, 1.0 / dlen(ux));
-  const D3 ez = dmul(cdir, 1.0 / L);
+  if (!(rl > 1e-6 * L * dlen(cup))) return false;
+  f->right = dmul(rx, 1.0 / rl);
+  const D3 ux = dcross(f->right, cdir);
+  f->up = dmul(ux, 1.0 / dlen(ux));
+  f->ez = dmul(cdir, 1.0 / L);
   const double T = tan(fov * 0.5 * M_PI / 180.0), A = (double)W / (double)H;
   const double jx = Rg * 0.5 / W, jy = Rg * 0.5 / H;
   const double amax = (1.0 + jx) * T * A / L, bmax = (1.0 + jy) * T / L;
-  const double fz_min = 3.0 / sqrt(1.0 + amax * amax + bmax * bmax), fz_max = 3.0;
-  const double rho = 0.02 * Rg * 1.001;
+  f->L = L; f->T = T; f->A = A; f->jx = jx; f->jy = jy;
+  f->fz_min = 3.0 / sqrt(1.0 + amax * amax + bmax * bmax);
+  f->fz_max = 3.0;
+  f->rho = 0.02 * Rg * 1.001;
+  return true;
+}
+
+void root_points(const float* lo, const float* hi, D3 pts[8]) {
+  double m = 0.0;
+  for (int k = 0; k < 3; ++k) m = fmax(m, fmax(fabs((double)lo[k]), fabs((double)hi[k])));
+  m = 1e-4 * m + 1e-6;
+  for (int i = 0; i < 8; ++i)
+    pts[i] = {(i & 1 ? hi[0] + m : lo[0] - m), (i & 2 ? hi[1] + m : lo[1] - m), (i & 4 ? hi[2] + m : lo[2] - m)};
+}
+
+bool light_points(const pt_area_light& li, D3 pts[8]) {
+  const D3 nr = d3(li.normal);
+  const double nl = dlen(nr);
+  if (!(nl > 0.0)) return false;
+  const D3 nn = dmul(nr, 1.0 / nl);
+  const D3 basis = fabs(nn.y) < 0.999 ? D3{0, 1, 0} : D3{1, 0, 0};
+  const D3 lr = dmul(dcross(nn, basis), 1.0 / dlen(dcross(nn, basis)));
+  const D3 lu = dcross(lr, nn);
+  double h0 = fabs((double)li.size[0]) * 0.5, h1 = fabs((double)li.size[1]) * 0.5;
+  const D3 pos = d3(li.position);
+  const double pm = fmax(fmax(fabs(pos.x), fabs(pos.y)), fabs(pos.z));
+  if (fabs(fabs(nn.y) - 0.999) < 1e-4) h0 = h1 = fmax(h0, h1) * 1.41422;
+  h0 = h0 * 1.0001 + 1e-4 * pm + 1e-6;
+  h1 = h1 * 1.0001 + 1e-4 * pm + 1e-6;
+  if (!(h0 < 1e30 && h1 < 1e30)) return false;
+  for (int i = 0; i < 4; ++i) {
+    const D3 c = dadd(dadd(pos, dmul(lr, i & 1 ? h0 : -h0)), dmul(lu, i & 2 ? h1 : -h1));
+    const double th = 1e-4 * (pm + h0 + h1) + 1e-6;
+    pts[2 * i] = dadd(c, dmul(nn, th));
+    pts[2 * i + 1] = dadd(c, dmul(nn, -th));
+  }
+  return true;
+}
+
+struct Projected {
+  double sx[8], sy[8], z[8];
+  double sx0, sx1, sy0, sy1, z0, z1;
+};
+bool project(const CullFrame& f, const D3* pts, int np, Projected* o) {
+  o->sx0 = o->sy0 = o->z0 = INFINITY;
+  o->sx1 = o->sy1 = o->z1 = -INFINITY;
+  for (int i = 0; i < np; ++i) {
+    const D3 r = dsub(pts[i], f.cpos);
+    const double X = ddot(r, f.right), Y = ddot(r, f.up), Z = ddot(r, f.ez);
+    if (!(Z > 1e-4 * (1.0 + dlen(r)))) return false;
+    o->sx[i] = X / Z; o->sy[i] = Y / Z; o->z[i] = Z;
+    o->sx0 = fmin(o->sx0, X / Z); o->sx1 = fmax(o->sx1, X / Z);
+    o->sy0 = fmin(o->sy0, Y / Z); o->sy1 = fmax(o->sy1, Y / Z);
+    o->z0 = fmin(o->z0, Z); o->z1 = fmax(o->z1, Z);
+  }
+  return true;
+}
+
+struct RectD {
+  double x0, x1, y0, y1, del, mx, my;
+};
+RectD object_rect(const CullFrame& f, const Projected& p, int W, int H) {
+  const double dd = fmax(fmax(fabs(1.0 / p.z0 - 1.0 / f.fz_min), fabs(1.0 / p.z0 - 1.0 / f.fz_max)),
+                         fmax(fabs(1.0 / p.z1 - 1.0 / f.fz_min), fabs(1.0 / p.z1 - 1.0 / f.fz_max)));
+  RectD r;
+  r.del = f.rho * dd;
+  r.x0 = -(p.sx1 + r.del) * f.L / (f.T * f.A); r.x1 = -(p.sx0 - r.del) * f.L / (f.T * f.A);
+  r.y0 = -(p.sy1 + r.del) * f.L / f.T; r.y1 = -(p.sy0 - r.del) * f.L / f.T;
+  r.mx = 2.0 / W + 1e-4 * (1.0 + fabs(r.x0) + fabs(r.x1));
+  r.my = 2.0 / H + 1e-4 * (1.0 + fabs(r.y0) + fabs(r.y1));
+  return r;
+}
+
+bool rect_floats(const CullFrame& f, RectD r, float* o) {
+  r.x0 -= f.jx + r.mx; r.x1 += f.jx + r.mx; r.y0 -= f.jy + r.my; r.y1 += f.jy + r.my;
+  if (!(r.x0 == r.x0 && r.x1 == r.x1 && r.y0 == r.y0 && r.y1 == r.y1)) return false;
+  o[0] = nextafterf((float)r.x0, -INFINITY); o[1] = nextafterf((float)r.x1, INFINITY);
+  o[2] = nextafterf((float)r.y0, -INFINITY); o[3] = nextafterf((float)r.y1, INFINITY);
+  return true;
+}
+
+bool object_footprint(const CullFrame& f, const Projected& p, int np, int W, int H, float* o) {
+  const RectD r = object_rect(f, p, W, H);
+  float pub[4];
+  if (!rect_floats(f, r, pub)) return false;
+  auto sq_range = [](double lo, double hi, double* mn, double* mx) {
+    *mn = lo <= 0.0 && hi >= 0.0 ? 0.0 : fmin(lo * lo, hi * hi);
+    *mx = fmax(lo * lo, hi * hi);
+  };
+  double a0, a1, b0, b1;
+  sq_range(p.sx0 - r.del, p.sx1 + r.del, &a0, &a1);
+  sq_range(p.sy0 - r.del, p.sy1 + r.del, &b0, &b1);
+  const double fz_lo = fmax(f.fz_min, 3.0 / sqrt(1.0 + a1 + b1)), fz_hi = fmin(f.fz_max, 3.0 / sqrt(1.0 + a0 + b0));
+  if (!(fz_lo <= fz_hi)) return false;
+  double px[32], py[32];
+  const double kx = f.L / (f.T * f.A), ky = f.L / f.T;
+  for (int i = 0; i < np; ++i) {
+    const double w = 1.0 / p.z[i];
+    const double d = f.rho * fmax(fabs(w - 1.0 / fz_lo), fabs(w - 1.0 / fz_hi));
+    const double cx = -p.sx[i] * kx, cy = -p.sy[i] * ky;
+    const double ex = d * kx + f.jx + r.mx, ey = d * ky + f.jy + r.my;
+    for (int k = 0; k < 4; ++k) {
+      px[4 * i + k] = cx + (k & 1 ? ex : -ex);
+      py[4 * i + k] = cy + (k & 2 ? ey : -ey);
+      if (!(fabs(px[4 * i + k]) < 1e30 && fabs(py[4 * i + k]) < 1e30)) return false;
+    }
+  }
+  const int n = 4 * np;
+  double x0 = INFINITY, x1 = -INFINITY, y0 = INFINITY, y1 = -INFINITY;
+  for (int i = 0; i < n; ++i) {
+    x0 = fmin(x0, px[i]); x1 = fmax(x1, px[i]);
+    y0 = fmin(y0, py[i]); y1 = fmax(y1, py[i]);
+  }
+  o[0] = fmaxf(pub[0], nextafterf((float)x0, -INFINITY)); o[1] = fminf(pub[1], nextafterf((float)x1, INFINITY));
+  o[2] = fmaxf(pub[2], nextafterf((float)y0, -INFINITY)); o[3] = fminf(pub[3], nextafterf((float)y1, INFINITY));
+  for (int k = 0; k < ptd::kFootprintPlanes; ++k) { o[4 + 3 * k] = 0.0f; o[5 + 3 * k] = 0.0f; o[6 + 3 * k] = 1.0f; }
+  int idx[32];
+  for (int i = 0; i < n; ++i) idx[i] = i;
+  for (int i = 1; i < n; ++i)
+    for (int j = i; j > 0 && (px[idx[j]] < px[idx[j - 1]] || (px[idx[j]] == px[idx[j - 1]] && py[idx[j]] < py[idx[j - 1]])); --j) {
+      const int t = idx[j]; idx[j] = idx[j - 1]; idx[j - 1] = t;
+    }
+  auto turn = [&](int a, int b, int c) { return (px[b] - px[a]) * (py[c] - py[a]) - (py[b] - py[a]) * (px[c] - px[a]); };
+  int hull[66], m = 0;
+  for (int i = 0; i < n; ++i) {
+    while (m >= 2 && turn(hull[m - 2], hull[m - 1], idx[i]) <= 0.0) --m;
+    hull[m++] = idx[i];
+  }
+  for (int i = n - 2, t = m + 1; i >= 0; --i) {
+    while (m >= t && turn(hull[m - 2], hull[m - 1], idx[i]) <= 0.0) --m;
+    hull[m++] = idx[i];
+  }
+  --m;
+  if (m < 3) return true;
+  double len[ptd::kFootprintPlanes] = {};
+  for (int e = 0; e < m; ++e) {
+    const int u = hull[e], v = hull[(e + 1) % m];
+    const double dx = px[v] - px[u], dy = py[v] - py[u];
+    const double l = sqrt(dx * dx + dy * dy);
+    if (!(l > 0.0) || fabs(dx) <= 1e-9 * l || fabs(dy) <= 1e-9 * l) continue;
+    const double a = dy / l, b = -dx / l, c = a * px[u] + b * py[u];
+    const float af = (float)a, bf = (float)b;
+    const float cf = nextafterf((float)(c + 4e-6 + 2e-6 * fabs(c)), INFINITY);
+    if (!(af == af && bf == bf && cf == cf)) continue;
+    int k = 0;
+    for (int t = 1; t < ptd::kFootprintPlanes; ++t)
+      if (len[t] < len[k]) k = t;
+    if (l <= len[k]) continue;
+    len[k] = l;
+    o[4 + 3 * k] = af; o[5 + 3 * k] = bf; o[6 + 3 * k] = cf;
+  }
+  return true;
+}
+
+void sure_none(float* o) {
+  o[0] = 1.0f; o[1] = -1.0f; o[2] = 1.0f; o[3] = -1.0f;
+  for (int k = 0; k < ptd::kFootprintPlanes; ++k) { o[4 + 3 * k] = 0.0f; o[5 + 3 * k] = 0.0f; o[6 + 3 * k] = -1.0f; }
+}
+
+void light_sure(const CullFrame& f, const pt_area_light& li, int W, int H, double Rg, float* o) {
+  sure_none(o);
+  for (int k = 0; k < 3; ++k)
+    if (!isfinite(li.intensity[k])) return;
+  const D3 nr = d3(li.normal);
+  const double nl = dlen(nr);
+  if (!(nl >= 0.02 && nl < 1e6)) return;
+  const D3 nn = dmul(nr, 1.0 / nl);
+  if (fabs(fabs(nn.y) - 0.999) < 1e-4) return;
+  const D3 basis = fabs(nn.y) < 0.999 ? D3{0, 1, 0} : D3{1, 0, 0};
+  const D3 lr = dmul(dcross(nn, basis), 1.0 / dlen(dcross(nn, basis)));
+  const D3 lu = dcross(lr, nn);
+  if (!(li.size[0] > 0.0f && li.size[1] > 0.0f)) return;
+  const double h0 = (double)li.size[0] * 0.5, h1 = (double)li.size[1] * 0.5;
+  const D3 pos = d3(li.position);
+  const double pm = fmax(fmax(fabs(pos.x), fabs(pos.y)), fabs(pos.z));
+  const double far = dlen(dsub(pos, f.cpos)) + h0 + h1;
+  if (!(far < 1e6)) return;
+  const double off = 0.02 * Rg * 1.001 * M_SQRT2;
+  const double cosmin = (fabs(ddot(nn, dsub(pos, f.cpos))) - off) / (far + off);
+  if (!(cosmin >= 0.05)) return;
+  const double shrink = 1e-4 * (pm + h0 + h1 + far) + 1e-6;
+  const double g0 = h0 * 0.9999 - shrink, g1 = h1 * 0.9999 - shrink;
+  if (!(g0 > 0.0 && g1 > 0.0)) return;
+  D3 pts[4];
+  const int order[4] = {0, 1, 3, 2};
+  for (int i = 0; i < 4; ++i) {
+    const int k = order[i];
+    pts[i] = dadd(dadd(pos, dmul(lr, k & 1 ? g0 : -g0)), dmul(lu, k & 2 ? g1 : -g1));
+  }
+  Projected p;
+  if (!project(f, pts, 4, &p)) return;
+  auto sq_range = [](double lo, double hi, double* mn, double* mx) {
+    *mn = lo <= 0.0 && hi >= 0.0 ? 0.0 : fmin(lo * lo, hi * hi);
+    *mx = fmax(lo * lo, hi * hi);
+  };
+  double a0, a1, b0, b1;
+  sq_range(p.sx0, p.sx1, &a0, &a1);
+  sq_range(p.sy0, p.sy1, &b0, &b1);
+  const double fz_lo = fmax(f.fz_min, 3.0 / sqrt(1.0 + a1 + b1)), fz_hi = fmin(f.fz_max, 3.0 / sqrt(1.0 + a0 + b0));
+  if (!(fz_lo <= fz_hi)) return;
+  double e = 0.0;
+  for (int i = 0; i < 4; ++i) {
+    const double w = 1.0 / p.z[i];
+    e = fmax(e, f.rho * fmax(fabs(w - 1.0 / fz_lo), fabs(w - 1.0 / fz_hi)));
+  }
+  const double kx = f.L / (f.T * f.A), ky = f.L / f.T;
+  double qx[4], qy[4], x0 = INFINITY, x1 = -INFINITY, y0 = INFINITY, y1 = -INFINITY;
+  for (int i = 0; i < 4; ++i) {
+    qx[i] = -p.sx[i] * kx; qy[i] = -p.sy[i] * ky;
+    x0 = fmin(x0, qx[i]); x1 = fmax(x1, qx[i]); y0 = fmin(y0, qy[i]); y1 = fmax(y1, qy[i]);
+  }
+  const double ex = e * kx + f.jx + 2.0 / W + 1e-4 * (1.0 + fabs(x0) + fabs(x1));
+  const double ey = e * ky + f.jy + 2.0 / H + 1e-4 * (1.0 + fabs(y0) + fabs(y1));
+  if (!(ex < 1e30 && ey < 1e30 && fabs(x0) < 1e30 && fabs(x1) < 1e30 && fabs(y0) < 1e30 && fabs(y1) < 1e30)) return;
+  double turn[4], area = 0.0;
+  for (int i = 0; i < 4; ++i) {
+    const int j = (i + 1) % 4, k = (i + 2) % 4;
+    turn[i] = (qx[j] - qx[i]) * (qy[k] - qy[j]) - (qy[j] - qy[i]) * (qx[k] - qx[j]);
+    area += qx[i] * qy[j] - qx[j] * qy[i];
+  }
+  const double sg = area > 0.0 ? 1.0 : -1.0;
+  for (int i = 0; i < 4; ++i)
+    if (!(sg * turn[i] > 0.0)) return;
+  float out[ptd::kFootprintFloats];
+  out[0] = nextafterf((float)(x0 + ex), INFINITY); out[1] = nextafterf((float)(x1 - ex), -INFINITY);
+  out[2] = nextafterf((float)(y0 + ey), INFINITY); out[3] = nextafterf((float)(y1 - ey), -INFINITY);
+  for (int i = 0; i < 4; ++i) {
+    const int j = (i + 1) % 4;
+    const double dx = sg * (qx[j] - qx[i]), dy = sg * (qy[j] - qy[i]);
+    const double l = sqrt(dx * dx + dy * dy);
+    if (!(l > 0.0)) return;
+    const double a = dy / l, b = -dx / l, c = a * qx[i] + b * qy[i];
+    const float af = (float)a, bf = (float)b;
+    const float cf = nextafterf((float)(c - (fabs(a) * ex + fabs(b) * ey) - (4e-6 + 2e-6 * fabs(c))), -INFINITY);
+    if (!(af == af && bf == bf && cf == cf)) return;
+    out[4 + 3 * i] = af; out[5 + 3 * i] = bf; out[6 + 3 * i] = cf;
+  }
+  for (int k = 0; k < ptd::kFootprintFloats; ++k) o[k] = out[k];
+}
+
+}
+
+int ptd::cull_sure(const float cam[16], int W, int H, const float* lo, const float* hi, const pt_area_light* lights,
+                   int n_lights, float* sure, int max_sure, double Rg) {
+  CullFrame f;
+  if (n_lights < 0 || n_lights > max_sure || !cull_frame(cam, W, H, Rg, &f)) return -1;
   int n = 0;
-  auto add_object = [&](const D3* pts, int np) -> bool {
-    double sx0 = INFINITY, sx1 = -INFINITY, sy0 = INFINITY, sy1 = -INFINITY, z0 = INFINITY, z1 = -INFINITY;
-    for (int i = 0; i < np; ++i) {
-      const D3 r = dsub(pts[i], cpos);
-      const double X = ddot(r, right), Y = ddot(r, up), Z = ddot(r, ez);
-      if (!(Z > 1e-4 * (1.0 + dlen(r)))) return false;
-      sx0 = fmin(sx0, X / Z); sx1 = fmax(sx1, X / Z);
-      sy0 = fmin(sy0, Y / Z); sy1 = fmax(sy1, Y / Z);
-      z0 = fmin(z0, Z); z1 = fmax(z1, Z);
-    }
-    const double dd = fmax(fmax(fabs(1.0 / z0 - 1.0 / fz_min), fabs(1.0 / z0 - 1.0 / fz_max)),
-                           fmax(fabs(1.0 / z1 - 1.0 / fz_min), fabs(1.0 / z1 - 1.0 / fz_max)));
-    const double del = rho * dd;
-    double x0 = -(sx1 + del) * L / (T * A), x1 = -(sx0 - del) * L / (T * A);
-    double y0 = -(sy1 + del) * L / T, y1 = -(sy0 - del) * L / T;
-    const double mx = 2.0 / W + 1e-4 * (1.0 + fabs(x0) + fabs(x1)), my = 2.0 / H + 1e-4 * (1.0 + fabs(y0) + fabs(y1));
-    x0 -= jx + mx; x1 += jx + mx; y0 -= jy + my; y1 += jy + my;
-    if (!(x0 == x0 && x1 == x1 && y0 == y0 && y1 == y1)) return false;
-    float* o = rects + 4 * n++;
-    o[0] = nextafterf((float)x0, -INFINITY); o[1] = nextafterf((float)x1, INFINITY);
-    o[2] = nextafterf((float)y0, -INFINITY); o[3] = nextafterf((float)y1, INFINITY);
-    return true;
-  };
-  {
-    double m = 0.0;
-    for (int k = 0; k < 3; ++k) m = fmax(m, fmax(fabs((double)lo[k]), fabs((double)hi[k])));
-    m = 1e-4 * m + 1e-6;
-    D3 pts[8];
-    for (int i = 0; i < 8; ++i)
-      pts[i] = {(i & 1 ? hi[0] + m : lo[0] - m), (i & 2 ? hi[1] + m : lo[1] - m), (i & 4 ? hi[2] + m : lo[2] - m)};
-    if (!add_object(pts, 8)) return -1;
-  }
   for (int l = 0; l < n_lights; ++l) {
-    const pt_area_light& li = lights[l];
-    const D3 nr = d3(li.normal);
-    const double nl = dlen(nr);
-    if (!(nl > 0.0)) return -1;
-    const D3 nn = dmul(nr, 1.0 / nl);
-    const D3 basis = fabs(nn.y) < 0.999 ? D3{0, 1, 0} : D3{1, 0, 0};
-    const D3 lr = dmul(dcross(nn, basis), 1.0 / dlen(dcross(nn, basis)));
-    const D3 lu = dcross(lr, nn);
-    double h0 = fabs((double)li.size[0]) * 0.5, h1 = fabs((double)li.size[1]) * 0.5;
-    const D3 pos = d3(li.position);
-    const double pm = fmax(fmax(fabs(pos.x), fabs(pos.y)), fabs(pos.z));
-    if (fabs(fabs(nn.y) - 0.999) < 1e-4) h0 = h1 = fmax(h0, h1) * 1.41422;
-    h0 = h0 * 1.0001 + 1e-4 * pm + 1e-6;
-    h1 = h1 * 1.0001 + 1e-4 * pm + 1e-6;
-    if (!(h0 < 1e30 && h1 < 1e30)) return -1;
-    D3 pts[8];
-    for (int i = 0; i < 4; ++i) {
-      const D3 c = dadd(dadd(pos, dmul(lr, i & 1 ? h0 : -h0)), dmul(lu, i & 2 ? h1 : -h1));
-      const double th = 1e-4 * (pm + h0 + h1) + 1e-6;
-      pts[2 * i] = dadd(c, dmul(nn, th));
-      pts[2 * i + 1] = dadd(c, dmul(nn, -th));
-    }
-    if (!add_object(pts, 8)) return -1;
-  }
+    light_sure(f, lights[l], W, H, Rg, sure + kFootprintFloats * l);
+    const float* r = sure + kFootprintFloats * l;
+    n += r[0] <= r[1] && r[2] <= r[3] ? 1 : 0;
+  }
+  return n;
+}
+
+int ptd::cull_rects(const float cam[16], int W, int H, const float* lo, const float* hi, const pt_area_light* lights,
+                    int n_lights, float* rects, int max_rects, double Rg) {
+  CullFrame f;
+  if (n_lights < 0 || n_lights + 1 > max_rects || !cull_frame(cam, W, H, Rg, &f)) return -1;
+  int n = 0;
+  D3 pts[8];
+  Projected p;
+  root_points(lo, hi, pts);
+  if (!project(f, pts, 8, &p) || !rect_floats(f, object_rect(f, p, W, H), rects + 4 * n++)) return -1;
+  for (int l = 0; l < n_lights; ++l)
+    if (!light_points(lights[l], pts) || !project(f, pts, 8, &p) ||
+        !rect_floats(f, object_rect(f, p, W, H), rects + 4 * n++))
+      return -1;
+  return n;
+}
+
+int ptd::cull_footprints(const float cam[16], int W, int H, const float* lo, const float* hi,
+                         const pt_area_light* lights, int n_lights, float* foot, int max_foot, double Rg) {
+  CullFrame f;
+  if (n_lights < 0 || n_lights + 1 > max_foot || !cull_frame(cam, W, H, Rg, &f)) return -1;
+  int n = 0;
+  D3 pts[8];
+  Projected p;
+  root_points(lo, hi, pts);
+  if (!project(f, pts, 8, &p) || !object_footprint(f, p, 8, W, H, foot + kFootprintFloats * n++)) return -1;
+  for (int l = 0; l < n_lights; ++l)
+    if (!light_points(lights[l], pts) || !project(f, pts, 8, &p) ||
+        !object_footprint(f, p, 8, W, H, foot + kFootprintFloats * n++))
+      return -1;
   return n;
 }
 
@@ -117,4 +344,31 @@
   return PT_OK;
 }
 
-}
+int pt_primary_cull_footprints(const float cam[16], int w, int h, const float root_min[3], const float root_max[3],
+                               const pt_area_light* lights, int n_lights, double radius_bound, float* footprints,
+                               int max_footprints, int* n_footprints) {
+  if (!cam || !root_min || !root_max || !footprints || !n_footprints || (n_lights > 0 && !lights))
+    return fail(PT_ERR_INVALID, "null argument");
+  if (max_footprints < 1) return fail(PT_ERR_INVALID, "max_footprints must be >= 1");
+  const double R = radius_bound < 0.0 ? ptd::kCullTightR : radius_bound;
+  if (!(R <= ptd::kGaussR)) return fail(PT_ERR_INVALID, "radius bound above 13.25");
+  *n_footprints = ptd::cull_footprints(cam, w, h, root_min, root_max, lights, n_lights, footprints, max_footprints, R);
+  return PT_OK;
+}
+
+int pt_primary_cull_sure(const float cam[16], int w, int h, const float root_min[3], const float root_max[3],
+                         const pt_area_light* lights, int n_lights, double radius_bound, float* regions,
+                         int max_regions, int* n_sure) {
+  if (!cam || !root_min || !root_max || !regions || !n_sure || (n_lights > 0 && !lights))
+    return fail(PT_ERR_INVALID, "null argument");
+  const double R = radius_bound < 0.0 ? ptd::kCullTightR : radius_bound;
+  if (!(R <= ptd::kGaussR)) return fail(PT_ERR_INVALID, "radius bound above 13.25");
+  float foot[ptd::kMaxCullObjects * ptd::kFootprintFloats];
+  *n_sure = -1;
+  if (n_lights <= max_regions &&
+      ptd::cull_footprints(cam, w, h, root_min, root_max, lights, n_lights, foot, ptd::kMaxCullObjects, R) >= 0)
+    *n_sure = ptd::cull_sure(cam, w, h, root_min, root_max, lights, n_lights, regions, max_regions, R);
+  return PT_OK;
+}
+
+}
diff --git a/discovering-path-tracer_amd/csrc/pt_cull.h b/discovering-path-tracer_amd/csrc/pt_cull.h
--- a/discovering-path-tracer_amd/csrc/pt_cull.h
+++ b/discovering-path-tracer_amd/csrc/pt_cull.h
@@ -21,4 +21,15 @@
                                                      const float* hi, const pt_area_light* lights, int n_lights,
                                                      float* rects, int max_rects, double Rg = kGaussR);
 
+constexpr int kMaxCullObjects = 8;
+constexpr int kFootprintPlanes = 4;
+constexpr int kFootprintFloats = 4 + 3 * kFootprintPlanes;
+__attribute__((visibility("hidden"))) int cull_footprints(const float cam[16], int W, int H, const float* lo,
+                                                          const float* hi, const pt_area_light* lights, int n_lights,
+                                                          float* foot, int max_foot, double Rg);
+
+__attribute__((visibility("hidden"))) int cull_sure(const float cam[16], int W, int H, const float* lo, const float* hi,
+                                                    const pt_area_light* lights, int n_lights, float* sure,
+                                                    int max_sure, double Rg);
+
 }
diff --git a/discovering-path-tracer_amd/csrc/pt_device.h b/discovering-path-tracer_amd/csrc/pt_device.h
--- a/discovering-path-tracer_amd/csrc/pt_device.h
+++ b/discovering-path-tracer_amd/csrc/pt_device.h
@@ -106,6 +106,9 @@
   uint32_t cube_under[6] = {};
   uint32_t cube_all = 0;
   int sweep_cube = 0;
+  int n_foot = 0;
+  int n_sure = 0;
+  const float* foot = nullptr;
 };
 constexpr int kMixShift = 24;
 constexpr int kMaxCullRects = 8;
diff --git a/discovering-path-tracer_amd/csrc/pt_group.cpp b/discovering-path-tracer_amd/csrc/pt_group.cpp
--- a/discovering-path-tracer_amd/csrc/pt_group.cpp
+++ b/discovering-path-tracer_amd/csrc/pt_group.cpp
@@ -606,6 +606,7 @@
 int wide_info(pt_group* g, int info[2]) { return pt_wide_info(g->m[0], info); }
 int sweep_info(pt_group* g, int* boxes, int* leaves) { return pt_sweep_info(g->m[0], boxes, leaves); }
 int sweep_walk(pt_group* g, int* walk) { return pt_sweep_walk(g->m[0], walk); }
+int cull_info(pt_group* g, int info[3]) { return pt_cull_info(g->m[0], info); }
 int last_launch_ms(pt_group* g, float* ms) { return pt_last_launch_ms(g->m[0], ms); }
 int launch_times_ms(pt_group* g, float* out, size_t max_n, size_t* n_out) {
   return pt_launch_times_ms(g->m[0], out, max_n, n_out);
diff --git a/discovering-path-tracer_amd/csrc/pt_group.h b/discovering-path-tracer_amd/csrc/pt_group.h
--- a/discovering-path-tracer_amd/csrc/pt_group.h
+++ b/discovering-path-tracer_amd/csrc/pt_group.h
@@ -41,6 +41,7 @@
 int wide_info(pt_group* g, int info[2]);
 int sweep_info(pt_group* g, int* boxes, int* leaves);
 int sweep_walk(pt_group* g, int* walk);
+int cull_info(pt_group* g, int info[3]);
 int last_launch_ms(pt_group* g, float* ms);
 int launch_times_ms(pt_group* g, float* out, size_t max_n, size_t* n_out);
 int launch_span_ms(pt_group* g, float* ms, size_t* n_out);
diff --git a/discovering-path-tracer_amd/ptamd.py b/discovering-path-tracer_amd/ptamd.py
--- a/discovering-path-tracer_amd/ptamd.py
+++ b/discovering-path-tracer_amd/ptamd.py
@@ -40,6 +40,7 @@
 PT_OPT_SWEEP_CUBE = 30
 PT_OPT_ADAPTIVE_WF = 31
 PT_OPT_RAYS_REFILL = 32
+PT_OPT_CULL_FOOTPRINT = 33
 RAYS_CLOSEST, RAYS_ANY = 0, 1
 RAY_DTYPE = np.dtype([("o", "<f4", 3), ("d", "<f4", 3), ("limit", "<f4"), ("reserved", "<u4")])
 HIT_DTYPE = np.dtype([("t", "<f4"), ("tri", "<i4"), ("u", "<f4"), ("v", "<f4"), ("n", "<f4", 3), ("reserved", "<u4")])
@@ -60,6 +61,7 @@
     "pt_dist_unique_id", "pt_dist_init", "pt_dist_run", "pt_dist_slot_floats", "pt_dist_finalize",
     "pt_dist_set_streams", "pt_dist_wait", "pt_dist_abort", "pt_create_multi", "pt_group_info",
     "pt_group_check", "pt_dist_info", "pt_mixed_info", "pt_sweep_info", "pt_sweep_walk",
+    "pt_primary_cull_footprints", "pt_primary_cull_sure", "pt_cull_info",
     "pt_denoise_default_params", "pt_guide_ray", "pt_render_guide", "pt_guide_device_ptr", "pt_read_guide",
     "pt_denoise", "pt_read_denoised", "pt_denoise_host",
     "pt_moments_device_ptr", "pt_read_moments", "pt_denoise_var_default_params", "pt_denoise_var",
@@ -169,6 +171,10 @@
             "pt_mixed_info": ([vp, ctypes.POINTER(ctypes.c_int)], i32),
             "pt_sweep_info": ([vp, ctypes.POINTER(ctypes.c_int), ctypes.POINTER(ctypes.c_int)], i32),
             "pt_sweep_walk": ([vp, ctypes.POINTER(ctypes.c_int)], i32),
+            "pt_cull_info": ([vp, vp], i32),
+            "pt_primary_cull_footprints": ([vp, i32, i32, vp, vp, vp, i32, ctypes.c_double, vp, i32,
+                                            ctypes.POINTER(i32)], i32),
+            "pt_primary_cull_sure": ([vp, i32, i32, vp, vp, vp, i32, ctypes.c_double, vp, i32, ctypes.POINTER(i32)], i32),
             "pt_partition_items": ([i32, i32, i32, i32, i32, vp, vp, i32, i32, vp, psz, vp, psz, vp], i32),
             "pt_dist_unique_id": ([vp, sz], i32), "pt_dist_init": ([vp, vp, i32, i32], i32),
             "pt_dist_run": ([vp, u32, i32, i32, vp, i32], i32), "pt_dist_slot_floats": ([vp, psz], i32),
@@ -424,6 +430,34 @@
     return (None if n.value < 0 else out[:n.value].copy()), float(u0.value)
 
 
+def primary_cull_footprints(camera_ubo, width, height, root_min, root_max, lights16, radius_bound=-1.0, max_footprints=8):
+    cam = np.ascontiguousarray(camera_ubo, np.float32).reshape(16)
+    lo = np.ascontiguousarray(root_min, np.float32).reshape(3)
+    hi = np.ascontiguousarray(root_max, np.float32).reshape(3)
+    l = np.ascontiguousarray(lights16, np.float32).reshape(-1)
+    out = np.zeros((max_footprints, 16), np.float32)
+    n = ctypes.c_int(0)
+    _check(lib().pt_primary_cull_footprints(cam.ctypes.data, width, height, lo.ctypes.data, hi.ctypes.data,
+                                            l.ctypes.data if l.size else None, l.size // 16, float(radius_bound),
+                                            out.ctypes.data, max_footprints, ctypes.byref(n)),
+           "pt_primary_cull_footprints")
+    return None if n.value < 0 else out[:n.value].copy()
+
+
+def primary_cull_sure(camera_ubo, width, height, root_min, root_max, lights16, radius_bound=-1.0):
+    cam = np.ascontiguousarray(camera_ubo, np.float32).reshape(16)
+    lo = np.ascontiguousarray(root_min, np.float32).reshape(3)
+    hi = np.ascontiguousarray(root_max, np.float32).reshape(3)
+    l = np.ascontiguousarray(lights16, np.float32).reshape(-1)
+    nl = l.size // 16
+    out = np.zeros((max(nl, 1), 16), np.float32)
+    n = ctypes.c_int(0)
+    _check(lib().pt_primary_cull_sure(cam.ctypes.data, width, height, lo.ctypes.data, hi.ctypes.data,
+                                      l.ctypes.data if l.size else None, nl, float(radius_bound), out.ctypes.data,
+                                      max(nl, 1), ctypes.byref(n)), "pt_primary_cull_sure")
+    return (None, -1) if n.value < 0 else (out[:nl].copy(), n.value)
+
+
 def write_image(path, rgba, width, height, fmt="png"):
     a = np.ascontiguousarray(rgba, np.float32).reshape(-1)
     if a.size != width * height * 4:
@@ -1050,6 +1084,11 @@
         _check(lib().pt_sweep_info(self._c, ctypes.byref(b), ctypes.byref(n)), "pt_sweep_info")
         return b.value, n.value
 
+    def cull_info(self):
+        info = (ctypes.c_int * 3)()
+        _check(lib().pt_cull_info(self._c, info), "pt_cull_info")
+        return info[0], info[1], info[2]
+
     def sweep_walk(self):
         w = ctypes.c_int(0)
         _check(lib().pt_sweep_walk(self._c, ctypes.byref(w)), "pt_sweep_walk")
diff --git a/include/pathtracer.h b/include/pathtracer.h
--- a/include/pathtracer.h
+++ b/include/pathtracer.h
@@ -255,6 +255,7 @@
 #define PT_OPT_SWEEP_CUBE 30
 #define PT_OPT_ADAPTIVE_WF 31
 #define PT_OPT_RAYS_REFILL 32
+#define PT_OPT_CULL_FOOTPRINT 33
 int pt_set_option(pt_context* ctx, int key, int value);
 int pt_last_kernel(pt_context* ctx, int* kernel);
 
@@ -264,6 +265,13 @@
 int pt_primary_cull_rects_r(const float camera_ubo[16], int width, int height, const float root_min[3],
                             const float root_max[3], const pt_area_light* lights, int n_lights, double radius_bound,
                             float* rects, int max_rects, int* n_rects, float* u0);
+int pt_primary_cull_footprints(const float camera_ubo[16], int width, int height, const float root_min[3],
+                               const float root_max[3], const pt_area_light* lights, int n_lights,
+                               double radius_bound, float* footprints, int max_footprints, int* n_footprints);
+int pt_primary_cull_sure(const float camera_ubo[16], int width, int height, const float root_min[3],
+                         const float root_max[3], const pt_area_light* lights, int n_lights, double radius_bound,
+                         float* regions, int max_regions, int* n_sure);
+int pt_cull_info(pt_context* ctx, int info[3]);
 
 int pt_set_stats_mode(pt_context* ctx, int enabled);
 int pt_get_stats(pt_context* ctx, pt_stats* out);
```

New measurement: 285,700, median of 6. +7.2%, better.
